# vlaxose/jstsp19

Measured on AMD Instinct MI355X. Metric: channel-estimates/sec (batched MC) at Nt=Nr=64,K=64; NMSE vs ref, higher is better.
Workload: dtype c32 (storage and results fp32 complex; big contractions as split-f16 MFMA with fp32 accumulation, fp32-equivalent); 1 GPU; proposed_algorithm approximate Imax=100, Nt=Nr=64 Nrf=8 K=64 L=8 (N=64 M=4096 Gr=64 G2=512); Imax=100, outputs=S,Y,convergence_error, pilots=per-trial (B per trial), parallelism=trials sharded, dp1

## Files before the change

jstsp19_amd/csrc/admm.hip:

```cpp
#include "common.h"
#include <algorithm>

namespace jstsp {

struct c2 { float2 a, b; };

__device__ __forceinline__ c2 ld2(const float2 *p, long long i)
{
    const float4 v = *reinterpret_cast<const float4 *>(p + i);
    c2 r; r.a = make_float2(v.x, v.y); r.b = make_float2(v.z, v.w); return r;
}
__device__ __forceinline__ void st2(float2 *p, long long i, const c2 &v)
{
    *reinterpret_cast<float4 *>(p + i) = make_float4(v.a.x, v.a.y, v.b.x, v.b.y);
}

__device__ __forceinline__ double wave_sum(double v)
{
    for (int o = 32; o > 0; o >>= 1) v += __shfl_xor(v, o);
    return v;
}

__device__ __forceinline__ double block_sum(double v, double *sh)
{
    v = wave_sum(v);
    __syncthreads();
    if ((threadIdx.x & 63) == 0) sh[threadIdx.x >> 6] = v;
    __syncthreads();
    return sh[0] + sh[1] + sh[2] + sh[3];
}

__global__ __launch_bounds__(256) void form_z_kernel(long long nm, const float2 *X, const float2 *V1,
                                                     const TrialParams *prm, float2 *Z)
{
    const int t = blockIdx.y;
    const TrialParams p = prm[t];
    const long long base = (long long)t * nm;
    const long long stride = (long long)gridDim.x * 256 * 2;
    const bool vec = (nm & 1) == 0;
    for (long long i = ((long long)blockIdx.x * 256 + threadIdx.x) * 2; i < nm; i += stride) {
        if (vec && i + 1 < nm) {
            const c2 x = ld2(X, base + i), v = ld2(V1, base + i);
            c2 z;
            z.a = make_float2(admm_z(p, x.a.x, v.a.x), admm_z(p, x.a.y, v.a.y));
            z.b = make_float2(admm_z(p, x.b.x, v.b.x), admm_z(p, x.b.y, v.b.y));
            st2(Z, base + i, z);
        } else {
            for (long long j = i; j < nm && j < i + 2; ++j) {
                const float2 x = X[base + j], v = V1[base + j];
                Z[base + j] = make_float2(admm_z(p, x.x, v.x), admm_z(p, x.y, v.y));
            }
        }
    }
}

__device__ __forceinline__ void upd_x_one(float2 &x, float2 &v1, const float2 v2, const float2 c,
                                          const float2 xs, const float2 y, const float2 sy,
                                          const float id, const TrialParams &p, float2 &k)
{
    const float tx = (y.x + c.x) + xs.x, ty = (y.y + c.y) + xs.y;
    const float bx = (v1.x + sy.x) + v2.x + mul2(p.rho, p.rho_lo, tx);
    const float by = (v1.y + sy.y) + v2.y + mul2(p.rho, p.rho_lo, ty);
    x = make_float2(bx * id, by * id);
    k = make_float2((fmaf(-p.irho, v2.x, x.x) - p.irho_lo * v2.x) - c.x, (fmaf(-p.irho, v2.y, x.y) - p.irho_lo * v2.y) - c.y);
    v1 = make_float2(admm_v1(p, v1.x, y.x, x.x), admm_v1(p, v1.y, y.y, x.y));
}

__global__ __launch_bounds__(256) void update_x_kernel(long long nm, float2 *X, float2 *V1,
                                                       const float2 *V2, const float2 *C,
                                                       const float2 *Xs, const float2 *Y,
                                                       const float2 *subY, const float *invD,
                                                       const TrialParams *prm, float2 *K)
{
    const int t = blockIdx.y;
    const TrialParams p = prm[t];
    const long long base = (long long)t * nm;
    const long long stride = (long long)gridDim.x * 256 * 2;
    const bool vec = (nm & 1) == 0;
    for (long long i = ((long long)blockIdx.x * 256 + threadIdx.x) * 2; i < nm; i += stride) {
        if (vec && i + 1 < nm) {
            c2 x, k, v1 = ld2(V1, base + i);
            const c2 v2 = ld2(V2, base + i), c = ld2(C, base + i), xs = ld2(Xs, base + i),
                     y = ld2(Y, base + i), sy = ld2(subY, base + i);
            const float2 id = *reinterpret_cast<const float2 *>(invD + base + i);
            upd_x_one(x.a, v1.a, v2.a, c.a, xs.a, y.a, sy.a, id.x, p, k.a);
            upd_x_one(x.b, v1.b, v2.b, c.b, xs.b, y.b, sy.b, id.y, p, k.b);
            st2(X, base + i, x); st2(V1, base + i, v1); st2(K, base + i, k);
        } else {
            for (long long j = i; j < nm && j < i + 2; ++j) {
                float2 x, k, v1 = V1[base + j];
                upd_x_one(x, v1, V2[base + j], C[base + j], Xs[base + j], Y[base + j], subY[base + j],
                          invD[base + j], p, k);
                X[base + j] = x; V1[base + j] = v1; K[base + j] = k;
            }
        }
    }
}

__device__ __forceinline__ void upd_c_one(const float2 x, const float2 xs, float2 &v2, float2 &c, const TrialParams &p)
{
    const float dx = x.x - xs.x, dy = x.y - xs.y;
    const float tx = fmaf(-p.irho, v2.x, dx) - p.irho_lo * v2.x, ty = fmaf(-p.irho, v2.y, dy) - p.irho_lo * v2.y;
    c = make_float2(mul2(p.c_coef, p.c_lo, tx), mul2(p.c_coef, p.c_lo, ty));
    const float ux = c.x - dx, uy = c.y - dy;
    v2 = make_float2(fmaf(p.rho, ux, v2.x) + p.rho_lo * ux, fmaf(p.rho, uy, v2.y) + p.rho_lo * uy);
}

__global__ __launch_bounds__(256) void update_c_kernel(long long nm, const float2 *X, const float2 *Xs,
                                                       float2 *V2, float2 *C, const TrialParams *prm)
{
    const int t = blockIdx.y;
    const TrialParams p = prm[t];
    const long long base = (long long)t * nm;
    const long long stride = (long long)gridDim.x * 256 * 2;
    const bool vec = (nm & 1) == 0;
    for (long long i = ((long long)blockIdx.x * 256 + threadIdx.x) * 2; i < nm; i += stride) {
        if (vec && i + 1 < nm) {
            const c2 x = ld2(X, base + i), xs = ld2(Xs, base + i);
            c2 v2 = ld2(V2, base + i), c;
            upd_c_one(x.a, xs.a, v2.a, c.a, p);
            upd_c_one(x.b, xs.b, v2.b, c.b, p);
            st2(C, base + i, c); st2(V2, base + i, v2);
        } else {
            for (long long j = i; j < nm && j < i + 2; ++j) {
                float2 v2 = V2[base + j], c;
                upd_c_one(X[base + j], Xs[base + j], v2, c, p);
                C[base + j] = c; V2[base + j] = v2;
            }
        }
    }
}

__global__ __launch_bounds__(256) void inv_d_kernel(long long nm, const float *Omega, float scale,
                                                    const TrialParams *prm, float *invD)
{
    const int t = blockIdx.y;
    const double add = (double)scale * ((double)prm[t].rho + (double)prm[t].rho_lo);
    const long long base = (long long)t * nm;
    const long long stride = (long long)gridDim.x * 256;
    for (long long i = (long long)blockIdx.x * 256 + threadIdx.x; i < nm; i += stride)
        invD[base + i] = (float)(1.0 / ((double)Omega[base + i] + add));
}

__device__ __forceinline__ float soft1(float v, float t)
{
    const float m = fmaxf(fabsf(v) - t, 0.f);
    return (v > 0.f) ? m : ((v < 0.f) ? -m : 0.f);
}

template <int NT>
__device__ __forceinline__ double block_sum_nt(double v, double *sh)
{
    v = wave_sum(v);
    __syncthreads();
    if ((threadIdx.x & 63) == 0) sh[threadIdx.x >> 6] = v;
    __syncthreads();
    double s = 0;
#pragma unroll
    for (int w = 0; w < NT / 64; ++w) s += sh[w];
    return s;
}
template <int NT>
__global__ __launch_bounds__(NT) void step_v_kernel(int g, const float2 *Res, const float2 *RRes,
                                                    float2 *V, float2 *S, const int32_t *rank,
                                                    int cnt, const TrialParams *prm, double *ce3,
                                                    int Imax, int it, float2 *RV, uint32_t *zero8)
{
    __shared__ double sh[NT / 64];
    const int t = blockIdx.x;
    const long long base = (long long)t * g;
    double num = 0, den_re = 0, den_im = 0, vprev = 0;
    constexpr int UN = 8;
    for (int i0 = threadIdx.x; i0 < g; i0 += NT * UN) {
        float2 r[UN], rr[UN], v[UN];
#pragma unroll
        for (int u = 0; u < UN; ++u) {
            const int i = min(i0 + u * NT, g - 1);
            r[u] = Res[base + i]; rr[u] = RRes[base + i]; v[u] = V[base + i];
        }
#pragma unroll
        for (int u = 0; u < UN; ++u)
            if (i0 + u * NT < g) {
                num += (double)r[u].x * r[u].x + (double)r[u].y * r[u].y;
                den_re += (double)r[u].x * rr[u].x + (double)r[u].y * rr[u].y;
                den_im += (double)r[u].x * rr[u].y - (double)r[u].y * rr[u].x;
                vprev += (double)v[u].x * v[u].x + (double)v[u].y * v[u].y;
            }
    }
    num = block_sum_nt<NT>(num, sh);
    den_re = block_sum_nt<NT>(den_re, sh);
    den_im = block_sum_nt<NT>(den_im, sh);
    vprev = block_sum_nt<NT>(vprev, sh);
    const double dd = den_re * den_re + den_im * den_im;
    const float ax = (float)(num * den_re / dd);
    const float ay = (float)(-num * den_im / dd);
    const float thr = prm[t].tauS_rho;
    for (int i0 = threadIdx.x; i0 < g; i0 += NT * UN) {
        float2 r[UN], v[UN], rr[UN], rv[UN];
        int rk[UN];
#pragma unroll
        for (int u = 0; u < UN; ++u) {
            const int i = min(i0 + u * NT, g - 1);
            r[u] = Res[base + i]; v[u] = V[base + i];
            if (RV) { rr[u] = RRes[base + i]; rv[u] = RV[base + i]; }
            rk[u] = rank ? rank[base + i] : 0;
        }
#pragma unroll
        for (int u = 0; u < UN; ++u) {
            const int i = i0 + u * NT;
            if (i >= g) break;
            float2 vn = v[u];
            vn.x += ax * r[u].x - ay * r[u].y;
            vn.y += ax * r[u].y + ay * r[u].x;
            V[base + i] = vn;
            if (RV) {
                float2 rn = rv[u];
                rn.x += ax * rr[u].x - ay * rr[u].y;
                rn.y += ax * rr[u].y + ay * rr[u].x;
                RV[base + i] = rn;
            }
            float2 sv = make_float2(soft1(vn.x, thr), soft1(vn.y, thr));
            if (rank && rk[u] >= cnt) sv = make_float2(0.f, 0.f);
            S[base + i] = sv;
        }
    }
    if (zero8 && threadIdx.x < 8) zero8[(size_t)threadIdx.x * gridDim.x + t] = 0u;
    if (ce3 && threadIdx.x == 0) {
        const double a2 = (double)ax * ax + (double)ay * ay;
        ce3[(long long)t * 3 * Imax + 2 * Imax + it] = a2 * num / vprev;
    }
}

__global__ __launch_bounds__(256) void soft_kernel(int g, const float2 *V, float2 *S,
                                                   const int32_t *rank, int cnt, const TrialParams *prm)
{
    const int t = blockIdx.y;
    const long long base = (long long)t * g;
    const float thr = prm[t].tauS_rho;
    for (int i = blockIdx.x * 256 + threadIdx.x; i < g; i += gridDim.x * 256) {
        const float2 v = V[base + i];
        float2 s = make_float2(soft1(v.x, thr), soft1(v.y, thr));
        if (rank && rank[base + i] >= cnt) s = make_float2(0.f, 0.f);
        S[base + i] = s;
    }
}

__global__ void rank_init_kernel(long long n, int32_t *rank)
{
    const long long i = (long long)blockIdx.x * 256 + threadIdx.x;
    if (i < n) rank[i] = 0x7fffffff;
}
__global__ void rank_scatter_kernel(int g, const int32_t *indx, int32_t *rank)
{
    const int t = blockIdx.y;
    const int p = blockIdx.x * 256 + threadIdx.x;
    if (p < g) {
        const int pos = indx[(long long)t * g + p] - 1;
        if (pos >= 0 && pos < g) atomicMin(&rank[(long long)t * g + pos], p);
    }
}

__global__ void ce_ratio_kernel(int batch, const float *lamV1, const float *lamV2, const float *lamX,
                                double *ce, int Imax, int it)
{
    const int t = blockIdx.x * 256 + threadIdx.x;
    if (t < batch) {
        ce[(long long)t * 3 * Imax + it] = (double)lamV1[t] / (double)lamX[t];
        ce[(long long)t * 3 * Imax + Imax + it] = (double)lamV2[t] / (double)lamX[t];
    }
}

static inline dim3 ew_grid(long long nm, int batch)
{
    long long blocks = (nm / 2 + 255) / 256;
    if (blocks < 1) blocks = 1;
    const long long cap = (2048 + batch - 1) / batch;
    if (blocks > cap) blocks = cap < 1 ? 1 : cap;
    return dim3((unsigned)blocks, (unsigned)batch);
}

int launch_form_z(jstsp_ctx *ctx, long long nm, int batch, const float2 *X, const float2 *V1,
                  const TrialParams *prm, float2 *Z)
{
    hipLaunchKernelGGL(form_z_kernel, ew_grid(nm, batch), dim3(256), 0, ctx->stream, nm, X, V1, prm, Z);
    JSTSP_HIP(hipGetLastError());
    return 0;
}
int launch_update_x(jstsp_ctx *ctx, long long nm, int batch, float2 *X, float2 *V1, const float2 *V2,
                    const float2 *C, const float2 *Xs, const float2 *Y, const float2 *subY,
                    const float *invD, const TrialParams *prm, float2 *K)
{
    hipLaunchKernelGGL(update_x_kernel, ew_grid(nm, batch), dim3(256), 0, ctx->stream, nm, X, V1, V2, C,
                       Xs, Y, subY, invD, prm, K);
    JSTSP_HIP(hipGetLastError());
    return 0;
}
int launch_update_c(jstsp_ctx *ctx, long long nm, int batch, const float2 *X, const float2 *Xs,
                    float2 *V2, float2 *C, const TrialParams *prm)
{
    hipLaunchKernelGGL(update_c_kernel, ew_grid(nm, batch), dim3(256), 0, ctx->stream, nm, X, Xs, V2, C,
                       prm);
    JSTSP_HIP(hipGetLastError());
    return 0;
}
int launch_step_v(jstsp_ctx *ctx, int g, int batch, const float2 *Res, const float2 *RRes, float2 *V,
                  float2 *S, const int32_t *rank, int cnt, const TrialParams *prm, double *ce3,
                  int Imax, int it, float2 *RV, int waves8, uint32_t *zero8)
{
    if (g >= 8192 && waves8)
        hipLaunchKernelGGL(step_v_kernel<512>, dim3(batch), dim3(512), 0, ctx->stream, g, Res, RRes, V, S, rank,
                           cnt, prm, ce3, Imax, it, RV, zero8);
    else if (g >= 8192)
        hipLaunchKernelGGL(step_v_kernel<1024>, dim3(batch), dim3(1024), 0, ctx->stream, g, Res, RRes, V, S, rank,
                           cnt, prm, ce3, Imax, it, RV, zero8);
    else
        hipLaunchKernelGGL(step_v_kernel<256>, dim3(batch), dim3(256), 0, ctx->stream, g, Res, RRes, V, S, rank,
                           cnt, prm, ce3, Imax, it, RV, zero8);
    JSTSP_HIP(hipGetLastError());
    return 0;
}
int launch_soft(jstsp_ctx *ctx, int g, int batch, const float2 *V, float2 *S, const int32_t *rank,
                int cnt, const TrialParams *prm)
{
    hipLaunchKernelGGL(soft_kernel, dim3((g + 255) / 256, batch), dim3(256), 0, ctx->stream, g, V, S,
                       rank, cnt, prm);
    JSTSP_HIP(hipGetLastError());
    return 0;
}
int launch_inv_d(jstsp_ctx *ctx, long long nm, int batch, const float *Omega, float scale,
                 const TrialParams *prm, float *invD)
{
    hipLaunchKernelGGL(inv_d_kernel, ew_grid(nm * 2, batch), dim3(256), 0, ctx->stream, nm, Omega, scale,
                       prm, invD);
    JSTSP_HIP(hipGetLastError());
    return 0;
}
int launch_rank_from_index(jstsp_ctx *ctx, int g, int batch, const int32_t *indx, int32_t *rank)
{
    const long long n = (long long)g * batch;
    hipLaunchKernelGGL(rank_init_kernel, dim3((unsigned)((n + 255) / 256)), dim3(256), 0, ctx->stream, n,
                       rank);
    hipLaunchKernelGGL(rank_scatter_kernel, dim3((g + 255) / 256, batch), dim3(256), 0, ctx->stream, g,
                       indx, rank);
    JSTSP_HIP(hipGetLastError());
    return 0;
}
__global__ __launch_bounds__(256) void eye_minus_kernel(int n, long long total, const float2 *Q, float2 *P)
{
    for (long long e = (long long)blockIdx.x * 256 + threadIdx.x; e < total; e += (long long)gridDim.x * 256) {
        const int r = (int)(e % ((long long)n * n));
        const float2 q = Q[e];
        P[e] = make_float2(((r % n) == (r / n) ? 1.f : 0.f) - q.x, -q.y);
    }
}
int launch_eye_minus(jstsp_ctx *ctx, int n, int count, const float2 *Q, float2 *P)
{
    const long long total = (long long)count * n * n;
    hipLaunchKernelGGL(eye_minus_kernel, dim3((unsigned)std::min<long long>((total + 255) / 256, 2048)), dim3(256), 0,
                       ctx->stream, n, total, Q, P);
    JSTSP_HIP(hipGetLastError());
    return 0;
}

int launch_ce_ratio(jstsp_ctx *ctx, int batch, const float *lamV1, const float *lamV2, const float *lamX,
                    double *ce, int Imax, int it)
{
    hipLaunchKernelGGL(ce_ratio_kernel, dim3((batch + 255) / 256), dim3(256), 0, ctx->stream, batch,
                       lamV1, lamV2, lamX, ce, Imax, it);
    JSTSP_HIP(hipGetLastError());
    return 0;
}

}
```

jstsp19_amd/csrc/common.h:

```cpp
#pragma once
#include <hip/hip_runtime.h>
#include <cstdint>
#include <cstdio>
#include <cstdarg>
#include <string>
#include <vector>
#include <map>
#include "../../include/jstsp.h"

namespace jstsp {

void set_error(const char *fmt, ...);

#define JSTSP_HIP(call)                                                                  \
    do {                                                                                 \
        hipError_t e_ = (call);                                                          \
        if (e_ != hipSuccess) {                                                          \
            jstsp::set_error("%s failed: %s (%s:%d)", #call, hipGetErrorString(e_),      \
                             __FILE__, __LINE__);                                        \
            return (int)e_;                                                              \
        }                                                                                \
    } while (0)

#define JSTSP_TRY(expr)                                                                  \
// ... 95 lines not shown
    const float ys = y + xs;
    const float s = (v1 + sy) + mul2(p.rho, p.rho_lo, ys) + mul2(p.omr, p.omr_lo, v2);
    return fmaf(s, rh, s * rl);
}
__device__ __forceinline__ void admm_invd(const TrialParams &p, float om, float &rh, float &rl)
{
    const float a = 2.f * p.rho, al = 2.f * p.rho_lo;
    const float dh = om + a;
    const float bb = dh - om;
    const float dl = ((om - (dh - bb)) + (a - bb)) + al;
    rh = __builtin_amdgcn_rcpf(dh);
    rl = rh * (fmaf(-dh, rh, 1.f) - dl * rh);
}
__device__ __forceinline__ float admm_k(const TrialParams &p, float x, float v2) { return fmaf(p.omir, v2, x) + p.omir_lo * v2; }
__device__ __forceinline__ float admm_v1(const TrialParams &p, float v1, float y, float x)
{
    const float d = y - x;
    return fmaf(p.rho, d, v1) + p.rho_lo * d;
}
__device__ __forceinline__ float admm_z(const TrialParams &p, float x, float v1) { return fmaf(-p.irho, v1, x) - p.irho_lo * v1; }
#endif
#endif

struct Arena {
    char *base = nullptr;
    size_t cap = 0, off = 0;
    int reserve(size_t bytes);
    void reset() { off = 0; }
    template <class T> T *get(size_t n) {
        size_t bytes = (n * sizeof(T) + 255) & ~size_t(255);
        if (off + bytes > cap) return nullptr;
        T *p = reinterpret_cast<T *>(base + off);
        off += bytes;
        return p;
    }
    void release();
};

struct ProfileSlot {
    int launches = 0;
    std::vector<std::pair<hipEvent_t, hipEvent_t>> pending;
    double total_ms = 0;
};

}

struct jstsp_ctx {
    int device = 0;
    hipStream_t stream = nullptr;
    bool own_stream = false;
    jstsp::Arena arena;
    bool profiling = false;
    std::map<std::string, jstsp::ProfileSlot> prof;
    std::vector<hipEvent_t> event_pool;
    int num_cus = 256;
    void *pinned = nullptr;
    size_t pinned_cap = 0, pinned_off = 0;
    hipEvent_t pinned_done = nullptr;
    bool pinned_pending = false;
    uint32_t *diag = nullptr;
    unsigned *lz_mismatch = nullptr;
    void *hpin = nullptr;
    size_t hpin_cap = 0;
    hipEvent_t hpin_done = nullptr;
    bool hpin_pending = false;
    int dict_block_hint = 0;
    int last_dict_block = 0;
    int fused_fallbacks = 0;
    float2 *unit = nullptr;
    double2 *unit64 = nullptr;
    jstsp_ctx *helper = nullptr;
    hipStream_t side[2] = {nullptr, nullptr};
    hipStream_t cu_stream[4] = {nullptr, nullptr, nullptr, nullptr};
    int cu_state = 0;
    hipStream_t bj_stream[3] = {nullptr, nullptr, nullptr};
    hipEvent_t bj_ev[6] = {nullptr, nullptr, nullptr, nullptr, nullptr, nullptr};
    hipEvent_t ev[10] = {nullptr, nullptr, nullptr, nullptr, nullptr, nullptr, nullptr, nullptr, nullptr, nullptr};
};

namespace jstsp {

struct GemmDesc {
    const float2 *A; long long sAt, sAi, sAk; int conjA;
    const float2 *B; long long sBt, sBk, sBj; int conjB;
    const float2 *B2;
    float2 *C; long long sCt; int ldc;
    const float2 *D; long long sDt; int ldd;
    float alpha, beta;
    int m, n, k, batch;
    int splitk; long long sCsplit;
    int epi;
    const TrialParams *prm;
    float2 *e_rw0, *e_w1, *e_w2, *e_w3;
    const float2 *e_r0, *e_r1, *e_r2, *e_r3;
    const float *e_f0;
    int epi_store_c;
    uint32_t *amax_x, *amax_v1, *amax_z;
    uint32_t *amax_out;
    int force_m64;
    float2 *C_lo;
    int herm_upper;
    int sa_mode;
    const float *sa_lr, *sa_lt;
    float sa_rho, sa_thr;
};
__device__ __forceinline__ float sadmm_den(float lr, float lt, float rho) { return fmaf(lr, lt, -rho); }
__device__ __forceinline__ float sadmm_dual1(float z, float r, float s, float rho) { return fmaf(rho, r - s, z); }
__device__ __forceinline__ float sadmm_soft1(float r, float z, float ir, float thr)
{
    const float v = fmaf(ir, z, r);
    const float m = fmaxf(fabsf(v) - thr, 0.f);
    return (v > 0.f) ? m : ((v < 0.f) ? -m : 0.f);
}
__device__ __forceinline__ float sadmm_rhs1(float z, float s, float a, float rho) { return fmaf(-rho, s, z) + a; }
enum { EPI_NONE = 0, EPI_UPDATE_C = 1, EPI_UPDATE_X = 2, EPI_SADMM = 3 };
enum { GEMM_MISC = 0, GEMM_CORRELATE = 1, GEMM_SYNTH = 2, GEMM_GRAM = 3 };
int launch_cgemm(jstsp_ctx *ctx, const GemmDesc &d, int tag = GEMM_MISC);

struct HPack {
    uint4 *data = nullptr;
    uint32_t *bmax = nullptr;
    int KS = 0, JT = 0, count = 0;
    long long st = 0;
};
struct HGemmDesc {
    const float2 *A; long long sAt, sAk;
    const uint32_t *amax;
    const uint4 *Bp; long long sPt;
    const uint32_t *bmax; int sbmax;
    int KS, JT;
    float2 *C; long long sCt; int ldc;
    int m, n, k, batch;
    int epi;
    const TrialParams *prm;
    const float2 *e_r0;
    float2 *e_rw0;
    uint32_t *amax_v2;
    const uint4 *Ap; long long sApt; int aKS;
    int herm_upper;
    int map_tb, map_tt;
};
int hermitian_fill_lower(jstsp_ctx *ctx, float2 *G, long long sGt, int n, int count);
int launch_hgram(jstsp_ctx *ctx, const float2 *Z, long long sZt, int rows, int cols, int count, int nsplit,
                 const uint32_t *amax, float2 *Gpart, const float2 *Z2 = nullptr,
                 const TrialParams *zprm = nullptr,
                 bool norm_only = false);
int launch_hgram3(jstsp_ctx *ctx, const float2 *X, const float2 *V1, long long sZt, int rows, int cols, int count, int nsplit,
                  const uint32_t *xmax, const uint32_t *vmax, const uint32_t *zmax, const TrialParams *prm, float2 *Gz,
                  float2 *Gx, float2 *Gv);
size_t hgemm_pack_bytes(int Kd, int J, int count);
bool hgemm_pair_shape(int m, int n, int batch);
int hgemm_absmax(jstsp_ctx *ctx, const float2 *X, long long n, long long sXt, int count, uint32_t *amax);
int hgemm_pack(jstsp_ctx *ctx, HPack &p, Arena &ar, const float2 *B, long long sBt, long long sBk, long long sBj,
               int conj, int Kd, int J, int count, long long n_contig, const uint32_t *bmax_known = nullptr);
int hgemm_repack(jstsp_ctx *ctx, const HPack &p, const float2 *B, long long sBt, long long sBk, long long sBj, int conj,
                 int Kd, int J, const uint32_t *bmax);
int launch_hgemm(jstsp_ctx *ctx, const HGemmDesc &d, const char *prof_name = nullptr);
bool use_hgemm(long long m, long long n, long long k);

enum { EIG_SVT_Q = 0, EIG_LMAX = 1, EIG_VECS = 2 };
int launch_eig(jstsp_ctx *ctx, int mode, int n, int batch, const float2 *Gpart, long long sGt,
               int nsplit, long long sGs, const TrialParams *prm, const float *tau,
               float2 *Q, float *lam_out, float2 *Vg);
bool eig_needs_global_v(int n);
int launch_eig_large(jstsp_ctx *ctx, int mode, int n, int batch, const float2 *Gpart, long long sGt, int nsplit,
                     long long sGs, const TrialParams *prm, const float *tau, float2 *Q, float *lam_out);
int launch_eig_fast(jstsp_ctx *ctx, int mode, int n, int batch, const float2 *Gpart, long long sGt, int nsplit,
                    long long sGs, const TrialParams *prm, const float *tau, float2 *Q, float *lam_out,
                    float2 *Uwarm, int warm);
int launch_eig128(jstsp_ctx *ctx, int n, int batch, const float2 *Gpart, long long sGt, int nsplit, long long sGs,
                  const TrialParams *prm, const float *tau, float2 *Q, float2 *Uwarm = nullptr, int warm = 0,
                  int max_sweeps = 16, float stop_level = 0.f);
int eig_fast_ne(int n);
struct LanczosWarm {
    float2 *x = nullptr;
    int *state = nullptr;
    unsigned *mismatch = nullptr;
    int ne = 0;
    int call = 0;
};
int lanczos_ne(int n);
int launch_lmax(jstsp_ctx *ctx, int n, int batch, const float2 *Gpart, long long sGt, int nsplit, long long sGs,
                float *lam_out, bool lanczos = false, const LanczosWarm *lw = nullptr, int first = 0);

int launch_form_z(jstsp_ctx *ctx, long long nm, int batch, const float2 *X, const float2 *V1,
                  const TrialParams *prm, float2 *Z);
int launch_update_x(jstsp_ctx *ctx, long long nm, int batch, float2 *X, float2 *V1,
                    const float2 *V2, const float2 *C, const float2 *Xs, const float2 *Y,
                    const float2 *subY, const float *invD, const TrialParams *prm, float2 *K);
int launch_update_c(jstsp_ctx *ctx, long long nm, int batch, const float2 *X, const float2 *Xs,
                    float2 *V2, float2 *C, const TrialParams *prm);
int launch_step_v(jstsp_ctx *ctx, int g, int batch, const float2 *Res, const float2 *RRes,
                  float2 *V, float2 *S, const int32_t *rank, int cnt, const TrialParams *prm,
                  double *ce3, int Imax, int it, float2 *RV = nullptr, int waves8 = 0,
                  uint32_t *zero8 = nullptr);
int launch_soft(jstsp_ctx *ctx, int g, int batch, const float2 *V, float2 *S, const int32_t *rank,
                int cnt, const TrialParams *prm);
int launch_inv_d(jstsp_ctx *ctx, long long nm, int batch, const float *Omega, float scale2rho,
                 const TrialParams *prm, float *invD);
int launch_rank_from_index(jstsp_ctx *ctx, int g, int batch, const int32_t *indx, int32_t *rank);
int launch_eye_minus(jstsp_ctx *ctx, int n, int count, const float2 *Q, float2 *P);
int launch_ce_ratio(jstsp_ctx *ctx, int batch, const float *lamV1, const float *lamV2,
                    const float *lamX, double *ce, int Imax, int it);

void prof_begin(jstsp_ctx *ctx, const char *name);
void prof_end(jstsp_ctx *ctx, const char *name);

}
```

jstsp19_amd/csrc/fused.hip:

```cpp
#include "solver_common.h"
#include <algorithm>
#include <cstdlib>
#include <cstdio>

namespace jstsp {
namespace {

typedef _Float16 half8 __attribute__((ext_vector_type(8)));
typedef _Float16 half4 __attribute__((ext_vector_type(4)));
typedef float f32x4 __attribute__((ext_vector_type(4)));

constexpr int FPAD = 128;

__device__ __host__ inline int fscale_exp(uint32_t amax_bits)
{
    const int be = (int)((amax_bits >> 23) & 0xff);
    if (be == 0 || be == 255) return 0;
    return 13 - (be - 127);
}
__device__ __forceinline__ void fsplit(float x, _Float16 &h, _Float16 &l)
{
    h = (_Float16)x;
    l = (_Float16)(x - (float)h);
}
typedef unsigned int u32x4 __attribute__((ext_vector_type(4)));
typedef unsigned int u32x2 __attribute__((ext_vector_type(2)));
__device__ __forceinline__ u32x4 negu(u32x4 u) { return u ^ 0x80008000u; }
template <class T> __device__ __forceinline__ T ldg(const void *base, uint32_t boff)
{
    return *reinterpret_cast<const T *>(reinterpret_cast<const char *>(base) + boff);
}
template <class T> __device__ __forceinline__ T ldg_nt(const void *base, uint32_t boff)
{
    return __builtin_nontemporal_load(reinterpret_cast<const T *>(reinterpret_cast<const char *>(base) + boff));
}
typedef float f32x2 __attribute__((ext_vector_type(2)));
__device__ __forceinline__ float2 ldg_nt2(const void *base, uint32_t boff)
{
    const f32x2 v = ldg_nt<f32x2>(base, boff);
    return make_float2(v.x, v.y);
}
__device__ __forceinline__ void stg_nt2(void *base, uint32_t boff, float2 v)
{
    __builtin_nontemporal_store(f32x2{v.x, v.y}, reinterpret_cast<f32x2 *>(reinterpret_cast<char *>(base) + boff));
}
template <class T> __device__ __forceinline__ void stg(void *base, uint32_t boff, T v)
{
    *reinterpret_cast<T *>(reinterpret_cast<char *>(base) + boff) = v;
}
__device__ __forceinline__ f32x4 mma(u32x4 a, u32x4 b, f32x4 c)
{
    return __builtin_amdgcn_mfma_f32_16x16x32_f16(__builtin_bit_cast(half8, a), __builtin_bit_cast(half8, b), c, 0, 0, 0);
}

__global__ __launch_bounds__(256) void pack_bf_kernel(const float2 *B, long long sBt, int G2, int M, const uint32_t *bmax,
                                                      int sbmax, uint4 *out, long long sOut)
{
    const int t = blockIdx.y;
    const int G8 = G2 >> 3;
    const long long per_tile = 32ll * G8;
    const long long idx = (long long)blockIdx.x * 256 + threadIdx.x;
    if (idx >= (long long)(M / 32) * per_tile) return;
    const int tile = (int)(idx / per_tile);
    int rem = (int)(idx % per_tile);
    const int g8 = rem % G8; rem /= G8;
    const int r = rem & 3, mq = rem >> 2;
    const int m = tile * 32 + 4 * mq + r;
    const float s = ldexpf(1.f, fscale_exp(bmax[(long long)t * sbmax]));
    half8 pl[4];
#pragma unroll
    for (int c = 0; c < 8; ++c) {
        const float2 x = B[(long long)t * sBt + (8 * g8 + c) + (long long)G2 * m];
        _Float16 h, l;
        fsplit(x.x * s, h, l); pl[0][c] = h; pl[1][c] = l;
        fsplit(x.y * s, h, l); pl[2][c] = h; pl[3][c] = l;
    }
    uint4 *o = out + (long long)t * sOut + (long long)tile * (16ll * G2);
    const int blk = g8 >> 1, g8i = g8 & 1;
#pragma unroll
    for (int p = 0; p < 4; ++p) o[(((long long)(blk * 4 + p) * 8 + mq) * 2 + g8i) * 4 + r] = *reinterpret_cast<uint4 *>(&pl[p]);
}

__global__ __launch_bounds__(256) void toeplitz_probe_kernel(const float2 *B, long long sBt, int G2, int M, uint32_t cand, uint32_t *mism)
{
    const uint32_t idx = blockIdx.x * 256u + threadIdx.x;
    uint32_t bad = 0;
    if (idx < (uint32_t)G2 * (uint32_t)M) {
        const int m = (int)(idx / (uint32_t)G2), g = (int)(idx - (uint32_t)m * (uint32_t)G2);
        const uint2 *b = reinterpret_cast<const uint2 *>(B) + (long long)blockIdx.y * sBt;
        const uint2 x = b[idx];
#pragma unroll
        for (int c = 0; c < 5; ++c) {
            const int gt = 16 << c, ld = g >> (4 + c);
            if (!((cand >> c) & 1u) || ld == 0 || m < ld) continue;
            const uint2 y = b[idx - (uint32_t)gt - (uint32_t)G2];
            if (x.x != y.x || x.y != y.y) bad |= 1u << c;
        }
    }
#pragma unroll
    for (int o = 32; o > 0; o >>= 1) bad |= __shfl_xor(bad, o);
    if ((threadIdx.x & 63) == 0 && (bad & ~__atomic_load_n(mism, __ATOMIC_RELAXED))) atomicOr(mism, bad);
}

__global__ __launch_bounds__(256) void toeplitz_verify_kernel(const float2 *B, long long sBt, int G2, int M, int c, uint32_t *mism)
{
    const uint32_t q = blockIdx.x * 256u + threadIdx.x;
    const uint32_t qpc = (uint32_t)G2 >> 2;
    uint32_t bad = 0;
    if (q < qpc * (uint32_t)M) {
        const int m = (int)(q / qpc), g = 4 * (int)(q - (uint32_t)m * qpc);
        const int gt = 16 << c, ld = g >> (4 + c);
        if (ld >= 1 && m >= ld) {
            const uint4 *b = reinterpret_cast<const uint4 *>(reinterpret_cast<const uint2 *>(B) + (long long)blockIdx.y * sBt);
            const uint32_t e = (uint32_t)g + (uint32_t)G2 * (uint32_t)m;
            const uint4 x0 = b[e >> 1], x1 = b[(e >> 1) + 1];
            const uint32_t f = e - (uint32_t)gt - (uint32_t)G2;
            const uint4 y0 = b[f >> 1], y1 = b[(f >> 1) + 1];
            if (x0.x != y0.x || x0.y != y0.y || x0.z != y0.z || x0.w != y0.w || x1.x != y1.x || x1.y != y1.y || x1.z != y1.z ||
                x1.w != y1.w)
                bad = 1u << c;
        }
    }
#pragma unroll
    for (int o = 32; o > 0; o >>= 1) bad |= __shfl_xor(bad, o);
    if ((threadIdx.x & 63) == 0 && (bad & ~__atomic_load_n(mism, __ATOMIC_RELAXED))) atomicOr(mism, bad);
}

__global__ __launch_bounds__(256) void pack_e_kernel(const float2 *B, long long sBt, int G2, int M, int gt, int ecols, int ehalo,
                                                     const uint32_t *bmax, int sbmax, uint4 *out, long long sOut)
{
    const int t = blockIdx.y;
    const int G8t = gt >> 3, L = G2 / gt;
    const long long idx = (long long)blockIdx.x * 256 + threadIdx.x;
    if (idx >= (long long)G8t * ecols) return;
    const int g8 = (int)(idx % G8t), j = (int)(idx / G8t);
    int row0 = 8 * g8, m = j - ehalo;
    bool live = true;
    if (m < 0) {
        const int jh = -m;
        int ld = 1;
        while (ld * (ld + 1) / 2 < jh) ++ld;
        live = ld < L;
        const int c = -(jh - ld * (ld - 1) / 2);
        m = c + ld; row0 += ld * gt;
    }
    const float s = ldexpf(1.f, fscale_exp(bmax[(long long)t * sbmax]));
    half8 pl[4];
#pragma unroll
    for (int c = 0; c < 8; ++c) {
        const float2 x = live ? B[(long long)t * sBt + (row0 + c) + (long long)G2 * m] : make_float2(0.f, 0.f);
        _Float16 h, l;
        fsplit(x.x * s, h, l); pl[0][c] = h; pl[1][c] = l;
        fsplit(x.y * s, h, l); pl[2][c] = h; pl[3][c] = l;
    }
    uint4 *o = out + (long long)t * sOut;
#pragma unroll
    for (int p = 0; p < 4; ++p) o[(long long)(p * G8t + g8) * ecols + j] = *reinterpret_cast<uint4 *>(&pl[p]);
}

__host__ __device__ inline int eswz(int x) { return (((x >> 1) & 3) << 1) | ((x >> 3) & 1); }

__global__ __launch_bounds__(256) void pack_e2_kernel(const float2 *B, long long sBt, int G2, int M, const uint32_t *bmax, int sbmax,
                                                      uint4 *out, long long sOut, float2 *Bdl)
{
    const int t = blockIdx.y;
    const int idx = blockIdx.x * 256 + threadIdx.x;
    if (idx < G2 * 8)
        Bdl[(long long)t * G2 * 8 + idx] = B[(long long)t * sBt + (idx >> 3) + (long long)G2 * (idx & 7)];
    if (idx >= (M + 8) * 8) return;
    const int o = idx & 7, cc = idx >> 3, m = cc - 7;
    const bool live = m >= 0 && m < M;
    const float s = ldexpf(1.f, fscale_exp(bmax[(long long)t * sbmax]));
    half8 pl[4];
#pragma unroll
    for (int c = 0; c < 8; ++c) {
        const float2 x = live ? B[(long long)t * sBt + (8 * o + c) + (long long)G2 * m] : make_float2(0.f, 0.f);
        _Float16 h, l;
        fsplit(x.x * s, h, l); pl[0][c] = h; pl[1][c] = l;
        fsplit(x.y * s, h, l); pl[2][c] = h; pl[3][c] = l;
    }
    uint4 *dst = out + (long long)t * sOut;
#pragma unroll
    for (int p = 0; p < 4; ++p) dst[((long long)p * (M + 8) + cc) * 8 + (o ^ eswz(cc))] = *reinterpret_cast<uint4 *>(&pl[p]);
}

__device__ __forceinline__ void xs_delta(const float2 *W, const float2 *Bdl, int G2, int m, int r, float2 *out)
{
    __shared__ float2 part[4][64];
    const int lane = threadIdx.x & 63, wv = threadIdx.x >> 6;
    const int g0 = 64 * (m + 1), cnt = G2 - g0;
    float2 a = make_float2(0.f, 0.f), a2 = a;
    const int per = (cnt + 15) / 16, lo = min(g0 + (4 * r + wv) * per, G2), hi = min(lo + per, G2);
    int g = lo;
    for (; g + 8 <= hi; g += 8) {
        float2 w[8], b[8];
#pragma unroll
        for (int u = 0; u < 8; ++u) { w[u] = W[lane + 64ll * (g + u)]; b[u] = Bdl[(g + u) * 8 + m]; }
#pragma unroll
        for (int u = 0; u < 8; u += 2) {
            a.x = fmaf(w[u].x, b[u].x, fmaf(-w[u].y, b[u].y, a.x)); a.y = fmaf(w[u].x, b[u].y, fmaf(w[u].y, b[u].x, a.y));
            a2.x = fmaf(w[u + 1].x, b[u + 1].x, fmaf(-w[u + 1].y, b[u + 1].y, a2.x));
            a2.y = fmaf(w[u + 1].x, b[u + 1].y, fmaf(w[u + 1].y, b[u + 1].x, a2.y));
        }
    }
    for (; g < hi; ++g) {
        const float2 w0 = W[lane + 64ll * g], b0 = Bdl[g * 8 + m];
        a.x = fmaf(w0.x, b0.x, fmaf(-w0.y, b0.y, a.x)); a.y = fmaf(w0.x, b0.y, fmaf(w0.y, b0.x, a.y));
    }
    part[wv][lane] = make_float2(a.x + a2.x, a.y + a2.y);
    __syncthreads();
    if (wv == 0) {
        const float2 p0 = part[0][lane], p1 = part[1][lane], p2 = part[2][lane], p3 = part[3][lane];
        out[lane + 64 * m] = make_float2((p0.x + p1.x) + (p2.x + p3.x), (p0.y + p1.y) + (p2.y + p3.y));
    }
}

__global__ __launch_bounds__(256) void pack_as_kernel(const float2 *W, long long sWt, int G2, const uint32_t *wmax, uint4 *out,
                                                      long long sOut, const float2 *Bd, long long sBd, float2 *XsD)
{
    const int t = blockIdx.y;
    if ((int)blockIdx.x >= G2 / 32) {
        const int e = (int)blockIdx.x - G2 / 32;
        xs_delta(W + (long long)t * sWt, Bd + (long long)t * sBd, G2, e >> 2, e & 3, XsD + (long long)t * 2048 + (e & 3) * 512);
        return;
    }
    const int idx = blockIdx.x * 256 + threadIdx.x;
    if (idx >= (G2 / 32) * 256) return;
    const int lane = idx & 63, nb = (idx >> 6) & 3, ks = idx >> 8;
    const int n = 16 * nb + (lane & 15), g0 = 32 * ks + 8 * (lane >> 4);
    const float s = ldexpf(1.f, fscale_exp(wmax[t]));
    half8 pl[4];
#pragma unroll
    for (int v = 0; v < 8; ++v) {
        const float2 x = W[(long long)t * sWt + n + 64ll * (g0 + v)];
        _Float16 h, l;
        fsplit(x.x * s, h, l); pl[0][v] = h; pl[1][v] = l;
        fsplit(x.y * s, h, l); pl[2][v] = h; pl[3][v] = l;
    }
    uint4 *o = out + (long long)t * sOut + (long long)((ks * 4 + nb) * 4) * 64 + lane;
#pragma unroll
    for (int p = 0; p < 4; ++p) o[p * 64] = *reinterpret_cast<uint4 *>(&pl[p]);
}

__global__ __launch_bounds__(256) void pack_wq_kernel(const float2 *Q, uint4 *out)
{
    const int t = blockIdx.x;
    const float2 *q = Q + (long long)t * 4096;
    for (int idx = threadIdx.x; idx < 512; idx += 256) {
        const int lane = idx & 63, nb = (idx >> 6) & 3, ks = idx >> 8;
        const int n = 16 * nb + (lane & 15), c0 = 32 * ks + 8 * (lane >> 4);
        half8 pl[4];
#pragma unroll
        for (int v = 0; v < 8; ++v) {
            const float2 x = q[n + 64 * (c0 + v)];
            _Float16 h, l;
            fsplit(((n == c0 + v) ? 1.f : 0.f) * 8192.f - x.x * 8192.f, h, l); pl[0][v] = h; pl[1][v] = l;
            fsplit(-x.y * 8192.f, h, l); pl[2][v] = h; pl[3][v] = l;
        }
        uint4 *o = out + (long long)t * 2048 + (long long)((ks * 4 + nb) * 4) * 64 + lane;
#pragma unroll
        for (int p = 0; p < 4; ++p) o[p * 64] = *reinterpret_cast<uint4 *>(&pl[p]);
    }
}

__global__ __launch_bounds__(256) void reduce_parts_kernel(const float4 *P, int parts, long long n4, float4 *out)
{
    const int t = blockIdx.y;
    const long long i = (long long)blockIdx.x * 256 + threadIdx.x;
    if (i >= n4) return;
    const float4 *p = P + (long long)t * parts * n4 + i;
    const float4 a0 = p[0];
    double ax = a0.x, ay = a0.y, az = a0.z, aw = a0.w;
    for (int s = 1; s < parts; ++s) {
        const float4 b = p[(long long)s * n4];
        ax += b.x; ay += b.y; az += b.z; aw += b.w;
    }
    out[(long long)t * n4 + i] = make_float4((float)ax, (float)ay, (float)az, (float)aw);
}
// ... 536 lines not shown
            ev2[s] = *reinterpret_cast<const float2 *>(sp_ + 2 * SFLD);  esy[s] = *reinterpret_cast<const float2 *>(sp_ + 3 * SFLD);
            eid[s] = *reinterpret_cast<const float *>(stag + SINV + (4 * q + s) * ICOL + c16 * 4);
        }
        __syncthreads();
        f32x4 xr = kh ? ar[1] : ar[0], xi = kh ? ai[1] : ai[0];
        {
            const f32x4 *x4 = reinterpret_cast<const f32x4 *>(pex);
            const f32x4 orr = x4[(w * 2 + 0) * 64 + l], oi = x4[(w * 2 + 1) * 64 + l];
            xr += orr; xi += oi;
        }
        half4 kf[4];
#pragma unroll
        for (int s = 0; s < 4; ++s) {
            const uint32_t ix = ebase + 512u * (uint32_t)(m0 + s);
            float2 xs = make_float2(xr[s] * sxs, xi[s] * sxs);
            const bool lead = m0 == 0 && kh == 0 && 4 * q + s < 2 * GB - 1;
            if (lead) {
                const float2 d0 = ldg<float2>(XsDt, ix), d1 = ldg<float2>(XsDt, ix + 4096), d2 = ldg<float2>(XsDt, ix + 8192),
                             d3 = ldg<float2>(XsDt, ix + 12288);
                xs.x += (d0.x + d1.x) + (d2.x + d3.x); xs.y += (d0.y + d1.y) + (d2.y + d3.y);
            }
            const float2 v2 = make_float2(admm_v2(prm, ev2[s].x, ex[s].x, xs.x), admm_v2(prm, ev2[s].y, ex[s].y, xs.y));
            float rh = eid[s], rl = 0.f;
            if (d.inv_is_omega) admm_invd(prm, eid[s], rh, rl);
            const float2 x = make_float2(admm_x2(prm, ev1[s].x, ey[s].x, esy[s].x, v2.x, xs.x, rh, rl),
                                         admm_x2(prm, ev1[s].y, ey[s].y, esy[s].y, v2.y, xs.y, rh, rl));
            const float2 kk = make_float2(admm_k(prm, x.x, v2.x), admm_k(prm, x.y, v2.y));
            const float2 v1 = make_float2(admm_v1(prm, ev1[s].x, ey[s].x, x.x), admm_v1(prm, ev1[s].y, ey[s].y, x.y));
            stg_nt2(V2t, ix, v2); stg_nt2(Xt, ix, x); stg_nt2(V1t, ix, v1);
            const float2 zn = make_float2(admm_z(prm, x.x, v1.x), admm_z(prm, x.y, v1.y));
            if (Zot) stg_nt2(Zot, ix, zn);
            if (Yot) stg(Yot, ix, ey[s]);
            if (lead) stg(Kft, ix, kk);
            v2mx = fmaxf(v2mx, fmaxf(fabsf(v2.x), fabsf(v2.y)));
            xmx = fmaxf(xmx, fmaxf(fabsf(x.x), fabsf(x.y)));
            v1mx = fmaxf(v1mx, fmaxf(fabsf(v1.x), fabsf(v1.y)));
            zmx = fmaxf(zmx, fmaxf(fabsf(zn.x), fabsf(zn.y)));
            kmx = fmaxf(kmx, fmaxf(fabsf(kk.x), fabsf(kk.y)));
            _Float16 h, lo;
            fsplit(kk.x * sk, h, lo); kf[0][s] = h; kf[1][s] = lo;
            fsplit(kk.y * sk, h, lo); kf[2][s] = h; kf[3][s] = lo;
        }
#pragma unroll
        for (int p = 0; p < 4; ++p)
            *reinterpret_cast<half4 *>(xch + ((nb * 6 + p) * 64 + l) * 16 + kh * 8) = kf[p];
        *reinterpret_cast<half4 *>(xch + ((nb * 6 + 4) * 64 + l) * 16 + kh * 8) = -kf[0];
        *reinterpret_cast<half4 *>(xch + ((nb * 6 + 5) * 64 + l) * 16 + kh * 8) = -kf[1];
        __syncthreads();
        const int tn = tile0 + min(i + 1, tpw - 1);
        typedef short s16x4 __attribute__((ext_vector_type(4)));
        typedef __attribute__((address_space(3))) s16x4 lds_s16x4;
        auto *lbase = (__attribute__((address_space(3))) unsigned char *)lds;
#pragma unroll
        for (int gb = 0; gb < GB; ++gb) {
            const int blk = GB * ws + gb, ld = blk >> 2, jp = 2 * (blk & 3);
            int cB = cB0 - ld;
            asm volatile("" : "+v"(cB));
            const uint32_t tr0 = (uint32_t)((i & 1) * EBUF) + cB * 128 + 16 * ((jp + ((c16 >> 1) & 1)) ^ eswz(cB)) + (c16 & 1) * 8;
            u32x4 bf[4];
#pragma unroll
            for (int p = 0; p < 4; ++p) {
                const uint32_t o_ = tr0 + p * EPL;
                const u32x2 lo_ = __builtin_bit_cast(u32x2, __builtin_amdgcn_ds_read_tr16_b64_v4i16((lds_s16x4 *)(lbase + o_)));
                const u32x2 hi_ = __builtin_bit_cast(u32x2, __builtin_amdgcn_ds_read_tr16_b64_v4i16((lds_s16x4 *)(lbase + o_ + 2048)));
                bf[p] = u32x4{lo_.x, lo_.y, hi_.x, hi_.y};
            }
#pragma unroll
            for (int n2 = 0; n2 < 4; ++n2) {
                const unsigned char *kp = xch + (n2 * 6 * 64 + l) * 16;
                u32x4 k0 = *reinterpret_cast<const u32x4 *>(kp), k1 = *reinterpret_cast<const u32x4 *>(kp + 1024);
                const u32x4 k2 = *reinterpret_cast<const u32x4 *>(kp + 2048), k3 = *reinterpret_cast<const u32x4 *>(kp + 3072);
                f32x4 tr = mma(bf[0], k0, f32x4{0.f, 0.f, 0.f, 0.f}), ti = mma(bf[0], k2, f32x4{0.f, 0.f, 0.f, 0.f});
                tr = mma(bf[0], k1, tr); ti = mma(bf[0], k3, ti);
                tr = mma(bf[1], k0, tr); ti = mma(bf[1], k2, ti);
                k0 = *reinterpret_cast<const u32x4 *>(kp + 4096); k1 = *reinterpret_cast<const u32x4 *>(kp + 5120);
                tr = mma(bf[2], k2, tr); ti = mma(bf[2], k0, ti);
                tr = mma(bf[2], k3, tr); ti = mma(bf[2], k1, ti);
                tr = mma(bf[3], k2, tr); ti = mma(bf[3], k0, ti);
                {
                    const int grp = 4 * gb + n2;
                    if (grp >= 6 && grp - 6 < 12) F64_STORE(grp - 6, (i + 1) & 1, rf[((grp - 6) >> 2) & 1][(grp - 6) & 3])
                    if (grp < 12) F64_LOAD(grp, tn, rf[(grp >> 2) & 1][grp & 3])
                }
                pr[gb][n2] += tr; pi[gb][n2] += ti;
                __builtin_amdgcn_sched_barrier(0);
            }
        }
        {
            constexpr int NG = 4 * GB;
#pragma unroll
            for (int pc = (NG > 6 ? NG - 6 : 0); pc < 12; ++pc) {
                if (pc >= NG) F64_LOAD(pc, tn, rf[(pc >> 2) & 1][pc & 3])
                F64_STORE(pc, (i + 1) & 1, rf[(pc >> 2) & 1][pc & 3])
            }
        }
        __builtin_amdgcn_sched_barrier(0);
        F64_WQLOAD()
        __syncthreads();
    }
#undef F64_LOAD
#undef F64_STORE
#undef F64_FLD
#undef F64_J
#undef F64_WQLOAD
    float2 *po = d.Ppart + ((long long)t * d.parts + part) * (64ll * G2);
#pragma unroll
    for (int gb = 0; gb < GB; ++gb)
#pragma unroll
        for (int n2 = 0; n2 < 4; ++n2)
#pragma unroll
            for (int s = 0; s < 4; ++s) {
                const int g = 16 * GB * w + 16 * gb + 4 * q + s;
                po[64ll * g + 16 * n2 + c16] = make_float2(pr[gb][n2][s] * sp, pi[gb][n2][s] * sp);
            }
#pragma unroll
    for (int o = 32; o > 0; o >>= 1) {
        kmx = fmaxf(kmx, __shfl_xor(kmx, o)); xmx = fmaxf(xmx, __shfl_xor(xmx, o)); v1mx = fmaxf(v1mx, __shfl_xor(v1mx, o));
        zmx = fmaxf(zmx, __shfl_xor(zmx, o)); v2mx = fmaxf(v2mx, __shfl_xor(v2mx, o));
    }
    if (l == 0) {
        if (d.kmax_out) atomicMax(&d.kmax_out[t], __float_as_uint(kmx));
        if (d.xmax) atomicMax(&d.xmax[t], __float_as_uint(xmx));
        if (d.v1max) atomicMax(&d.v1max[t], __float_as_uint(v1mx));
        if (d.zmax) atomicMax(&d.zmax[t], __float_as_uint(zmx));
        if (d.v2max) atomicMax(&d.v2max[t], __float_as_uint(v2mx));
        if (d.ovf && !(kmx * sk < 60000.f)) atomicOr(&d.ovf[t], 1u);
    }
}

}

bool fused_shape_ok(int N, int M, int G2, int parts)
{
    return N == 64 && G2 >= 128 && G2 <= 512 && G2 % 128 == 0 && parts > 0 && M % (32 * parts) == 0;
}

static void compact_dims(int M, int G2, int gt, int *ecols, int *ehalo)
{
    const int L = G2 / gt;
    *ehalo = ((L * (L - 1) / 2 + 3) / 4) * 4;
    *ecols = *ehalo + M;
}

size_t fused_bytes(int M, int G2, int nB, int batch, int parts)
{
    int ec, eh;
    compact_dims(M, G2, 16, &ec, &eh);
    return rnd256((size_t)nB * (M / 32) * 16 * G2 * sizeof(uint4)) + rnd256((size_t)batch * (G2 / 32) * 1024 * sizeof(uint4)) +
           rnd256((size_t)batch * parts * 64 * G2 * sizeof(float2)) + rnd256((size_t)batch * sizeof(uint32_t)) + rnd256((size_t)batch * 2048 * sizeof(uint4)) +
           rnd256((size_t)nB * 4 * (G2 / 16) * ec * sizeof(uint4)) + 5 * rnd256((size_t)batch * 512 * sizeof(float2)) +
           rnd256((size_t)nB * G2 * 8 * sizeof(float2)) + 512;
}

int fused_probe_toeplitz(jstsp_ctx *ctx, Arena &ar, const float2 *B, long long sBt, int G2, int M, int nB, int *gt)
{
    *gt = 0;
    uint32_t *flag = ar.get<uint32_t>(1);
    JSTSP_REQUIRE(flag, JSTSP_E_NOMEM, "fused pass: workspace exhausted");
    JSTSP_REQUIRE((long long)G2 * M < (1ll << 31), JSTSP_E_UNSUPPORTED, "fused pass: dictionary too large");
    uint32_t cand = 0;
    for (int c = 0; c < 5; ++c)
        if (G2 % (16 << c) == 0 && 2 * (16 << c) <= G2) cand |= 1u << c;
    const unsigned nblk = (unsigned)(((long long)G2 * M + 255) / 256);
    for (int step = 0; step < (nB > 1 ? 2 : 1) && cand; ++step) {
        JSTSP_HIP(hipMemsetAsync(flag, 0, sizeof(uint32_t), ctx->stream));
        if (step && sBt % 2 == 0)
            hipLaunchKernelGGL(toeplitz_verify_kernel, dim3((nblk + 3) / 4, nB), dim3(256), 0, ctx->stream, B, sBt, G2, M,
                               31 - __builtin_clz(cand), flag);
        else
            hipLaunchKernelGGL(toeplitz_probe_kernel, dim3(nblk, step ? nB : 1), dim3(256), 0, ctx->stream, B, sBt, G2, M, cand, flag);
        JSTSP_HIP(hipGetLastError());
        uint32_t bad = ~0u;
        JSTSP_HIP(hipMemcpyAsync(&bad, flag, sizeof(uint32_t), hipMemcpyDeviceToHost, ctx->stream));
        JSTSP_HIP(hipStreamSynchronize(ctx->stream));
        cand &= ~bad;
        cand &= cand ? (~cand + 1u) : 0u;
    }
    if (cand) *gt = 16 << (31 - __builtin_clz(cand));
    return 0;
}

__global__ __launch_bounds__(256) void toeplitz_gram_kernel(const float2 *B, long long sBt, int G2, int M, int gt, const float2 *G0,
                                                            const float2 *G0lo, float2 *G, float2 *Glo)
{
    const int t = blockIdx.y;
    const int idx = blockIdx.x * 256 + threadIdx.x;
    if (idx >= G2 * G2) return;
    const int r = idx % G2, c = idx / G2;
    const int ld = r / gt, g = r - ld * gt, l2 = c / gt, g2 = c - l2 * gt;
    if (ld > l2) return;
    const int d = l2 - ld;
    const float2 *b = B + (long long)t * sBt;
    const long long i0 = (long long)t * gt * G2 + g + (long long)gt * (d * gt + g2);
    double vr = (double)G0[i0].x + (G0lo ? (double)G0lo[i0].x : 0.0), vi = (double)G0[i0].y + (G0lo ? (double)G0lo[i0].y : 0.0);
    auto mac = [&](float2 x, float2 y, double sgn) {
        vr += sgn * ((double)x.x * y.x + (double)x.y * y.y);
        vi += sgn * ((double)x.y * y.x - (double)x.x * y.y);
    };
    for (int m = 0; m < d; ++m) mac(b[g + (long long)G2 * m], b[d * gt + g2 + (long long)G2 * m], -1.0);
    for (int u = M - ld; u < M; ++u) mac(b[g + (long long)G2 * u], b[g2 + (long long)G2 * (u - d)], -1.0);
    for (int m = 0; m < l2; ++m) mac(b[r + (long long)G2 * m], b[c + (long long)G2 * m], 1.0);
    if (r == c) vi = 0.0;
    const float hr = (float)vr, hi = (float)vi;
    float2 *o = G + (long long)t * G2 * G2;
    o[r + (long long)G2 * c] = make_float2(hr, hi);
    if (ld < l2) o[c + (long long)G2 * r] = make_float2(hr, -hi);
    if (Glo) {
        float2 *ol = Glo + (long long)t * G2 * G2;
        const float lr = (float)(vr - (double)hr), li = (float)(vi - (double)hi);
        ol[r + (long long)G2 * c] = make_float2(lr, li);
        if (ld < l2) ol[c + (long long)G2 * r] = make_float2(lr, -li);
    }
}

int toeplitz_gram_assemble(jstsp_ctx *ctx, const float2 *B, long long sBt, int G2, int M, int gt, int nB, const float2 *G0,
                           const float2 *G0lo, float2 *G, float2 *Glo)
{
    hipLaunchKernelGGL(toeplitz_gram_kernel, dim3((unsigned)((G2 * G2 + 255) / 256), nB), dim3(256), 0, ctx->stream, B, sBt, G2, M, gt,
                       G0, G0lo, G, Glo);
    JSTSP_HIP(hipGetLastError());
    return 0;
}

int fused_alloc(Arena &ar, FusedWS &f, int M, int G2, int nB, int batch, int parts, int gt, int v2)
{
    f.parts = parts;
    f.sBf = (long long)(M / 32) * 16 * G2;
    f.sAS = (long long)(G2 / 32) * 1024;
    f.gt = gt;
    f.v2 = (gt == 64 && v2) ? 1 : 0;
    if (f.v2) {
        f.ecols = M + 8; f.ehalo = 7;
        f.sEc = 4ll * f.ecols * 8;
        f.Ec = ar.get<uint4>((size_t)nB * f.sEc);
        f.XsD = ar.get<float2>((size_t)batch * 2048);
        f.Kf = ar.get<float2>((size_t)batch * 512);
        f.Bdl = ar.get<float2>((size_t)nB * G2 * 8);
        JSTSP_REQUIRE(f.XsD && f.Kf && f.Bdl, JSTSP_E_NOMEM, "fused pass: workspace exhausted");
    } else if (gt) {
        compact_dims(M, G2, gt, &f.ecols, &f.ehalo);
        f.sEc = 4ll * (gt / 8) * f.ecols;
        f.Ec = ar.get<uint4>((size_t)nB * f.sEc);
    } else
        f.Bf = ar.get<uint4>((size_t)nB * f.sBf);
    f.ASp = ar.get<uint4>((size_t)batch * f.sAS);
    f.Ppart = ar.get<float2>((size_t)batch * parts * 64 * G2);
    f.ovf = ar.get<uint32_t>(batch);
    f.Wqp = ar.get<uint4>((size_t)batch * 2048);
    JSTSP_REQUIRE((f.Bf || f.Ec) && f.ASp && f.Ppart && f.ovf && f.Wqp, JSTSP_E_NOMEM, "fused pass: workspace exhausted");
    return 0;
}

int fused_pack_b(jstsp_ctx *ctx, FusedWS &f, const float2 *B, long long sBt, int G2, int M, int nB, const uint32_t *bmax)
{
    f.Bsrc = B; f.sBsrc = sBt;
    if (f.v2) {
        hipLaunchKernelGGL(pack_e2_kernel, dim3((unsigned)((std::max(M + 8, G2) * 8 + 255) / 256), nB), dim3(256), 0, ctx->stream, B, sBt, G2, M,
                           bmax, 1, f.Ec, f.sEc, f.Bdl);
        JSTSP_HIP(hipGetLastError());
        f.sBdl = sBt ? (long long)G2 * 8 : 0;
        return 0;
    }
    if (f.gt) {
        const long long n = (long long)(f.gt / 8) * f.ecols;
        hipLaunchKernelGGL(pack_e_kernel, dim3((unsigned)((n + 255) / 256), nB), dim3(256), 0, ctx->stream, B, sBt, G2, M, f.gt,
                           f.ecols, f.ehalo, bmax, 1, f.Ec, f.sEc);
        JSTSP_HIP(hipGetLastError());
        return 0;
    }
    const long long n = (long long)(M / 32) * 16 * (G2 / 4);
    hipLaunchKernelGGL(pack_bf_kernel, dim3((unsigned)((n + 255) / 256), nB), dim3(256), 0, ctx->stream, B, sBt, G2, M, bmax, 1,
                       f.Bf, f.sBf);
    JSTSP_HIP(hipGetLastError());
    return 0;
}

int fused_pack_as(jstsp_ctx *ctx, const FusedWS &f, const float2 *W, long long sWt, int G2, int M, int batch, const uint32_t *wmax)
{
    hipLaunchKernelGGL(pack_as_kernel, dim3((G2 / 32) + (f.v2 ? 4 * (G2 / 64 - 1) : 0), batch), dim3(256), 0, ctx->stream, W, sWt, G2, wmax,
                       f.ASp, f.sAS, f.Bdl, f.sBdl, f.XsD);
    JSTSP_HIP(hipGetLastError());
    return 0;
}

template <int GB> static int launch_fused64(jstsp_ctx *ctx, const FusedDesc &d)
{
    const size_t sh = 2 * 20480 + 24576 + 8 * (4 * 16 * 128 + 16 * 80) + 16384;
    const int grid = ((d.batch + 7) / 8) * 8 * d.parts;
    JSTSP_HIP(hipFuncSetAttribute((const void *)fused_pass64_kernel<GB>, hipFuncAttributeMaxDynamicSharedMemorySize, (int)sh));
    hipLaunchKernelGGL((fused_pass64_kernel<GB>), dim3(grid), dim3(512), sh, ctx->stream, d);
    return 0;
}

template <int GB, bool YIN, bool TOEP> static int launch_fused_gb(jstsp_ctx *ctx, const FusedDesc &d)
{
    const size_t sh = (size_t)32 * (128 * GB * 8 + FPAD) + 24576;
    const int grid = ((d.batch + 7) / 8) * 8 * d.parts;
    JSTSP_HIP(hipFuncSetAttribute((const void *)fused_pass_kernel<GB, YIN, TOEP>, hipFuncAttributeMaxDynamicSharedMemorySize, (int)sh));
    hipLaunchKernelGGL((fused_pass_kernel<GB, YIN, TOEP>), dim3(grid), dim3(512), sh, ctx->stream, d);
    return 0;
}

template <bool YIN, bool TOEP> static int launch_fused_y(jstsp_ctx *ctx, const FusedDesc &d)
{
    switch (d.G2 / 128) {
    case 1: return launch_fused_gb<1, YIN, TOEP>(ctx, d);
    case 2: return launch_fused_gb<2, YIN, TOEP>(ctx, d);
    case 3: return launch_fused_gb<3, YIN, TOEP>(ctx, d);
    default: return launch_fused_gb<4, YIN, TOEP>(ctx, d);
    }
}

int launch_fused_pass(jstsp_ctx *ctx, const FusedDesc &d)
{
    JSTSP_REQUIRE(fused_shape_ok(64, d.M, d.G2, d.parts), JSTSP_E_UNSUPPORTED, "fused pass: shape");
    JSTSP_REQUIRE(d.Ec ? (d.gsh >= 4 && d.gsh <= 8) : d.Bf != nullptr, JSTSP_E_UNSUPPORTED, "fused pass: dictionary image");
    prof_begin(ctx, "fused_pass");
    int rc = 0;
    if (d.v2) {
// ... 39 lines not shown
```

jstsp19_amd/csrc/hgemm.hip:

```cpp
#include "solver_common.h"
#include <type_traits>

namespace jstsp {

typedef _Float16 half8 __attribute__((ext_vector_type(8)));
typedef float f32x16 __attribute__((ext_vector_type(16)));
typedef unsigned int u32x4 __attribute__((ext_vector_type(4)));

namespace {

constexpr int HBK = 32;
constexpr int FLUSH = 8;
constexpr float LO_SCALE = 1.f, LO_INV = 1.f;

__device__ __host__ inline int scale_exp(uint32_t amax_bits)
{
    const int be = (int)((amax_bits >> 23) & 0xff);
    if (be == 0 || be == 255) return 0;
    return 13 - (be - 127);
}

__device__ __forceinline__ void split2(float x, _Float16 &h, _Float16 &l)
{
    h = (_Float16)x;
    l = (_Float16)((x - (float)h) * LO_SCALE);
}

__global__ __launch_bounds__(256) void absmax_kernel(long long n2, const float *X, long long sXt, uint32_t *amax)
{
    const int t = blockIdx.y;
    const float *p = X + (long long)t * sXt;
    float m = 0.f;
    const bool vec = ((sXt & 3) == 0) && ((n2 & 3) == 0) && (((uintptr_t)X & 15) == 0);
    if (vec) {
        const float4 *p4 = reinterpret_cast<const float4 *>(p);
        for (long long i = (long long)blockIdx.x * 256 + threadIdx.x; i < n2 / 4; i += (long long)gridDim.x * 256) {
            const float4 v = p4[i];
            m = fmaxf(fmaxf(m, fmaxf(fabsf(v.x), fabsf(v.y))), fmaxf(fabsf(v.z), fabsf(v.w)));
        }
    } else {
        for (long long i = (long long)blockIdx.x * 256 + threadIdx.x; i < n2; i += (long long)gridDim.x * 256)
            m = fmaxf(m, fabsf(p[i]));
    }
    for (int o = 32; o > 0; o >>= 1) m = fmaxf(m, __shfl_xor(m, o));
    __shared__ float sm[4];
    if ((threadIdx.x & 63) == 0) sm[threadIdx.x >> 6] = m;
    __syncthreads();
    if (threadIdx.x == 0)
        atomicMax(&amax[t], __float_as_uint(fmaxf(fmaxf(sm[0], sm[1]), fmaxf(sm[2], sm[3]))));
}

__global__ __launch_bounds__(256) void pack_b_kernel(const float2 *B, long long sBt, long long sBk, long long sBj,
                                                     int conj, int Kd, int J, int KS, int JT, const uint32_t *bmax,
                                                     uint4 *out)
{
    const int t = blockIdx.y;
    const long long idx = (long long)blockIdx.x * 256 + threadIdx.x;
    if (idx >= (long long)JT * KS * 64) return;
    const int lane = (int)(idx & 63);
    const long long blk = idx >> 6;
    const int ks = (int)(blk % KS), jt = (int)(blk / KS);
    const int j = jt * 32 + (lane & 31), k0 = ks * 16 + 8 * (lane >> 5);
    const float s = ldexpf(1.f, scale_exp(bmax[t]));
    const float sg = conj ? -s : s;
    half8 rh, rl, ih, il;
#pragma unroll
    for (int v = 0; v < 8; ++v) {
        float2 x = make_float2(0.f, 0.f);
        if (j < J && k0 + v < Kd) x = B[(long long)t * sBt + (long long)(k0 + v) * sBk + (long long)j * sBj];
        _Float16 h, l;
        split2(x.x * s, h, l); rh[v] = h; rl[v] = l;
        split2(x.y * sg, h, l); ih[v] = h; il[v] = l;
    }
    uint4 *o = out + (((long long)t * JT + jt) * KS + ks) * 256 + lane;
    o[0] = *reinterpret_cast<uint4 *>(&rh);
    o[64] = *reinterpret_cast<uint4 *>(&rl);
    o[128] = *reinterpret_cast<uint4 *>(&ih);
    o[192] = *reinterpret_cast<uint4 *>(&il);
}

__device__ __forceinline__ half8 as_half8(uint4 u) { return *reinterpret_cast<half8 *>(&u); }
__device__ __forceinline__ half8 neg_half8(uint4 u)
{
    u.x ^= 0x80008000u; u.y ^= 0x80008000u; u.z ^= 0x80008000u; u.w ^= 0x80008000u;
    return *reinterpret_cast<half8 *>(&u);
}

__device__ __forceinline__ bool block_to_trial_tile(const HGemmDesc &d, int tiles, int &t, int &tile)
{
    const int bid = blockIdx.x;
    const int xcd = bid & 7, slot = bid >> 3;
    if (d.map_tb == 0) {
        t = (slot / tiles) * 8 + xcd;
        tile = slot % tiles;
        return t < d.batch;
    }
    const int per = d.map_tb * d.map_tt;
    const int nbt = (d.batch + d.map_tb - 1) / d.map_tb;
    const int blk = (slot / per) * 8 + xcd, w = slot % per;
    t = (blk % nbt) * d.map_tb + w % d.map_tb;
    tile = (blk / nbt) * d.map_tt + w / d.map_tb;
    return t < d.batch && tile < tiles;
}

template <int EPI, bool APACK, int WJ, bool EVEN = false>
__global__ __launch_bounds__(128 * WJ, WJ == 2 ? 2 : 2) void hgemm_kernel(HGemmDesc d, int tiles_i, int tiles_j)
{
    constexpr int STG = 1024 + 512 * WJ;
    constexpr int NA = (WJ == 2) ? 8 : 4;
    __shared__ uint4 smem[2 * STG];

    const int tiles = tiles_i * tiles_j;
    int t, rem;
    if (!block_to_trial_tile(d, tiles, t, rem)) return;
    const int ti = rem % tiles_i, tj = rem / tiles_i;
    const int i0 = ti * 64, j0 = tj * 32 * WJ;
    if (d.herm_upper && i0 >= j0 + 32 * WJ) return;

    const int tid = threadIdx.x, lane = tid & 63, wave = tid >> 6;
    const int wi = wave & 1, wj = wave >> 1;

    const int ea = scale_exp(d.amax[t]);
    const int eb = scale_exp(d.bmax[(long long)t * d.sbmax]);
    const float sa = ldexpf(1.f, ea);

    const int ai = tid & 63, akg = tid >> 6;
    const bool arow = (i0 + ai) < d.m;
    const float2 *abase = APACK ? nullptr : d.A + (long long)t * d.sAt;
    const float2 *pa = APACK ? nullptr : abase + (arow ? (i0 + ai) : 0) + (long long)(NA * akg) * d.sAk;
    const int a_slot = (WJ == 2) ? ((((ai >> 5) * 2 + (akg >> 1)) * 4) * 64) + (akg & 1) * 32 + (ai & 31)
                                 : ((((ai >> 5) * 2 + (akg >> 2)) * 4) * 64) + ((akg >> 1) & 1) * 32 + (ai & 31);
    const uint4 *pb = d.Bp + (long long)t * d.sPt + ((long long)(tj * WJ) * d.KS) * 256 + lane;
    const int nst = d.KS / 2;
    const int kfull = d.k / HBK;

    struct StgF { float2 a[NA]; uint4 b0, b1, b2, b3; };
    struct StgP { u32x4 a0, a1, a2, a3; uint4 b0, b1, b2, b3; };
    using Stg = typename std::conditional<APACK, StgP, StgF>::type;
    const uint4 *pbw = pb + ((long long)(wave >> 1) * d.KS + (wave & 1)) * 256;
    const uint4 *paw = APACK ? d.Ap + (long long)t * d.sApt + lane +
                                   ((long long)(ti * 2 + (wave >> 1)) * d.KS + (wave & 1)) * 256
                             : nullptr;
    const float sa_m = arow ? sa : 0.f;
    auto load = [&](int s_in, Stg &R) {
        const int s = EVEN ? (s_in < nst ? s_in : 0) : s_in;
        const uint4 *g = pbw + (long long)(2 * s) * 256;
        const u32x4 *gn = reinterpret_cast<const u32x4 *>(g);
        const u32x4 x0 = __builtin_nontemporal_load(gn), x1 = __builtin_nontemporal_load(gn + 64),
                    x2 = __builtin_nontemporal_load(gn + 128), x3 = __builtin_nontemporal_load(gn + 192);
        R.b0 = make_uint4(x0.x, x0.y, x0.z, x0.w); R.b1 = make_uint4(x1.x, x1.y, x1.z, x1.w);
        R.b2 = make_uint4(x2.x, x2.y, x2.z, x2.w); R.b3 = make_uint4(x3.x, x3.y, x3.z, x3.w);
        if constexpr (APACK) {
            const u32x4 *ga = reinterpret_cast<const u32x4 *>(paw + (long long)(2 * s) * 256);
            R.a0 = ga[0]; R.a1 = ga[64]; R.a2 = ga[128]; R.a3 = ga[192];
        } else {
            if (EVEN || s < kfull) {
#pragma unroll
                for (int v = 0; v < NA; ++v) R.a[v] = pa[(long long)(s * HBK + v) * d.sAk];
            } else {
                const int kbase = s * HBK + NA * akg;
#pragma unroll
                for (int v = 0; v < NA; ++v) {
                    const bool ok = kbase + v < d.k;
                    const float2 *p = ok ? pa + (long long)(s * HBK + v) * d.sAk : abase;
                    const float2 x = *p;
                    R.a[v] = ok ? x : make_float2(0.f, 0.f);
                }
            }
        }
    };
    auto store = [&](const Stg &R, uint4 *buf) {
        uint4 *o = buf + 1024 + wave * 256 + lane;
        o[0] = R.b0; o[64] = R.b1; o[128] = R.b2; o[192] = R.b3;
        if constexpr (APACK) {
            u32x4 *q = reinterpret_cast<u32x4 *>(buf + wave * 256 + lane);
            q[0] = R.a0; q[64] = R.a1; q[128] = R.a2; q[192] = R.a3;
        } else {
            half8 rh = {0}, rl = {0}, ih = {0}, il = {0};
#pragma unroll
            for (int v = 0; v < NA; ++v) {
                _Float16 h, l;
                split2(R.a[v].x * sa_m, h, l); rh[v] = h; rl[v] = l;
                split2(R.a[v].y * sa_m, h, l); ih[v] = h; il[v] = l;
            }
            if constexpr (WJ == 2) {
                uint4 *q = buf + a_slot;
                q[0] = *reinterpret_cast<uint4 *>(&rh);
                q[64] = *reinterpret_cast<uint4 *>(&rl);
                q[128] = *reinterpret_cast<uint4 *>(&ih);
                q[192] = *reinterpret_cast<uint4 *>(&il);
            } else {
                uint2 *q = reinterpret_cast<uint2 *>(buf + a_slot) + (akg & 1);
                q[0] = *reinterpret_cast<uint2 *>(&rh);
                q[2 * 64] = *reinterpret_cast<uint2 *>(&rl);
                q[2 * 128] = *reinterpret_cast<uint2 *>(&ih);
                q[2 * 192] = *reinterpret_cast<uint2 *>(&il);
            }
        }
    };

    f32x16 re_h = {0}, re_l = {0}, im_h = {0}, im_l = {0};
    f32x16 Lre = {0}, Lim = {0};
    auto fold = [&]() {
#pragma unroll
        for (int r = 0; r < 16; ++r) {
            Lre[r] += re_h[r] + re_l[r] * LO_INV;
            Lim[r] += im_h[r] + im_l[r] * LO_INV;
            re_h[r] = 0.f; re_l[r] = 0.f; im_h[r] = 0.f; im_l[r] = 0.f;
        }
    };
    auto compute = [&](const uint4 *buf) {
#pragma unroll
        for (int ks = 0; ks < 2; ++ks) {
            const uint4 *fa = buf + ((wi * 2 + ks) * 4) * 64 + lane;
            const uint4 *fb = buf + 1024 + ((wj * 2 + ks) * 4) * 64 + lane;
            const uint4 uar_h = fa[0], uar_l = fa[64], uai_h = fa[128], uai_l = fa[192];
            const half8 br_h = as_half8(fb[0]), br_l = as_half8(fb[64]), bi_h = as_half8(fb[128]), bi_l = as_half8(fb[192]);
            const half8 ar_h = as_half8(uar_h), ar_l = as_half8(uar_l), ai_h = as_half8(uai_h), ai_l = as_half8(uai_l);
            const half8 nai_h = neg_half8(uai_h), nai_l = neg_half8(uai_l);
            re_h = __builtin_amdgcn_mfma_f32_32x32x16_f16(br_h, ar_h, re_h, 0, 0, 0);
            re_l = __builtin_amdgcn_mfma_f32_32x32x16_f16(br_l, ar_h, re_l, 0, 0, 0);
            im_h = __builtin_amdgcn_mfma_f32_32x32x16_f16(bi_h, ar_h, im_h, 0, 0, 0);
            im_l = __builtin_amdgcn_mfma_f32_32x32x16_f16(bi_l, ar_h, im_l, 0, 0, 0);
            re_h = __builtin_amdgcn_mfma_f32_32x32x16_f16(bi_h, nai_h, re_h, 0, 0, 0);
            re_l = __builtin_amdgcn_mfma_f32_32x32x16_f16(br_h, ar_l, re_l, 0, 0, 0);
// ... 690 lines not shown
            const float2 *p = px + (long long)(s * HBK) * rows;
#pragma unroll
            for (int u = 0; u < 8; ++u) { R.x[u] = p[(long long)u * rows]; R.v[u] = p[(long long)u * rows + dv]; }
        } else {
            const int kbase = kbeg + s * HBK + 8 * akg;
#pragma unroll
            for (int u = 0; u < 8; ++u) {
                const int kk = min(kbase + u, cols - 1);
                const long long ix = base + (long long)kk * rows;
                float2 a = X[ix], b = V1[ix];
                if (kbase + u >= kend) { a = make_float2(0.f, 0.f); b = make_float2(0.f, 0.f); }
                R.x[u] = a; R.v[u] = b;
            }
        }
    };
    auto put = [&](uint4 *panel, const float2 *val, float sc) {
        half8 rh, rl, ih, il;
#pragma unroll
        for (int u = 0; u < 8; ++u) {
            _Float16 h, l;
            split2(val[u].x * sc, h, l); rh[u] = h; rl[u] = l + l;
            split2(val[u].y * sc, h, l); ih[u] = h; il[u] = l + l;
        }
        uint4 *q = panel + a_slot;
        q[0] = *reinterpret_cast<uint4 *>(&rh);
        q[64] = *reinterpret_cast<uint4 *>(&rl);
        q[128] = *reinterpret_cast<uint4 *>(&ih);
        q[192] = *reinterpret_cast<uint4 *>(&il);
    };
    auto put_h = [&](uint4 *panel, const float2 *val, float sc) {
        half8 rh, ih;
#pragma unroll
        for (int u = 0; u < 8; ++u) { rh[u] = (_Float16)(val[u].x * sc); ih[u] = (_Float16)(val[u].y * sc); }
        uint4 *q = panel + a_slot;
        q[0] = *reinterpret_cast<uint4 *>(&rh);
        q[128] = *reinterpret_cast<uint4 *>(&ih);
    };
    auto store = [&](const Stg &R) {
        float2 z[8];
#pragma unroll
        for (int u = 0; u < 8; ++u)
            z[u] = make_float2(fmaf(-ir, R.v[u].x, R.x[u].x) - irl * R.v[u].x, fmaf(-ir, R.v[u].y, R.x[u].y) - irl * R.v[u].y);
        if constexpr (NH) { put_h(smem, R.x, sx); put_h(smem + 1024, R.v, sv); }
        else { put(smem, R.x, sx); put(smem + 1024, R.v, sv); }
        put(smem + 2048, z, sz);
    };
    f32x16 re[3], im[3];
#pragma unroll
    for (int g = 0; g < 3; ++g)
#pragma unroll
        for (int r = 0; r < 16; ++r) { re[g][r] = 0.f; im[g][r] = 0.f; }
    auto compute = [&]() {
#pragma unroll
        for (int g = 0; g < 3; ++g) {
            const uint4 *buf = smem + g * 1024;
#pragma unroll
            for (int ks = 0; ks < 2; ++ks) {
                const uint4 *fi = buf + ((wi * 2 + ks) * 4) * 64 + lane;
                const uint4 *fj = buf + ((wj * 2 + ks) * 4) * 64 + lane;
                const half8 ir_h = as_half8(fi[0]), ii_h = as_half8(fi[128]);
                const uint4 ujr_h = fj[0], ujr_l = fj[64], uji_h = fj[128], uji_l = fj[192];
                const half8 jr_h = as_half8(ujr_h), jr_l = as_half8(ujr_l), ji_h = as_half8(uji_h), ji_l = as_half8(uji_l);
                const half8 nji_h = neg_half8(uji_h), nji_l = neg_half8(uji_l);
                re[g] = __builtin_amdgcn_mfma_f32_32x32x16_f16(jr_h, ir_h, re[g], 0, 0, 0);
                im[g] = __builtin_amdgcn_mfma_f32_32x32x16_f16(jr_h, ii_h, im[g], 0, 0, 0);
                re[g] = __builtin_amdgcn_mfma_f32_32x32x16_f16(ji_h, ii_h, re[g], 0, 0, 0);
                im[g] = __builtin_amdgcn_mfma_f32_32x32x16_f16(nji_h, ir_h, im[g], 0, 0, 0);
                if (NH && g < 2) continue;
                re[g] = __builtin_amdgcn_mfma_f32_32x32x16_f16(jr_l, ir_h, re[g], 0, 0, 0);
                im[g] = __builtin_amdgcn_mfma_f32_32x32x16_f16(jr_l, ii_h, im[g], 0, 0, 0);
                re[g] = __builtin_amdgcn_mfma_f32_32x32x16_f16(ji_l, ii_h, re[g], 0, 0, 0);
                im[g] = __builtin_amdgcn_mfma_f32_32x32x16_f16(nji_l, ir_h, im[g], 0, 0, 0);
            }
        }
    };
    if (nst > 0) {
        if constexpr (EVEN) {
            Stg R0, R1;
            load(0, R0);
            load(1, R1);
            store(R0);
            __syncthreads();
            for (int s = 0; s < nst; s += 2) {
                load(s + 2, R0);
                compute();
                __syncthreads();
                store(R1);
                __syncthreads();
                load(s + 3, R1);
                compute();
                __syncthreads();
                store(R0);
                __syncthreads();
            }
        } else {
            Stg R;
            load(0, R);
            store(R);
            __syncthreads();
            for (int s = 0; s < nst; ++s) {
                load(min(s + 1, nst - 1), R);
                compute();
                __syncthreads();
                store(R);
                __syncthreads();
            }
        }
    }
#pragma unroll
    for (int g = 0; g < 3; ++g) herm_symmetrize(re[g], im[g], reinterpret_cast<float2 *>(smem), wi, wj, lane);
    const int gi = wi * 32 + (lane & 31);
    const long long po = ((long long)t * nsplit + split) * rows * rows;
    if (gi < rows) {
        const float ax = ldexpf(1.f, -2 * ex), av = ldexpf(1.f, -2 * ev), az = ldexpf(1.f, -2 * ez);
#pragma unroll
        for (int r = 0; r < 16; ++r) {
            const int gj = wj * 32 + (r & 3) + 8 * (r >> 2) + 4 * (lane >> 5);
            if (gj < rows) {
                const long long o = po + gi + (long long)gj * rows;
                Gx[o] = make_float2(re[0][r] * ax, im[0][r] * ax);
                Gv[o] = make_float2(re[1][r] * av, im[1][r] * av);
                Gz[o] = make_float2(re[2][r] * az, im[2][r] * az);
            }
        }
    }
}

}

bool use_hgemm(long long m, long long n, long long k)
{
    const int mode = tune().h2;
    if (mode == 0) return false;
    if (mode >= 2) return true;
    return m * n * k >= (1ll << 22) && k >= 64 && n >= 64;
}

size_t hgemm_pack_bytes(int Kd, int J, int count)
{
    const size_t KS = 4 * (size_t)((Kd + 63) / 64), JT = 4 * (size_t)((J + 127) / 128);
    return rnd256((size_t)count * JT * KS * 4096) + rnd256((size_t)count * sizeof(uint32_t));
}

int hgemm_absmax(jstsp_ctx *ctx, const float2 *X, long long n, long long sXt, int count, uint32_t *amax)
{
    JSTSP_HIP(hipMemsetAsync(amax, 0, (size_t)count * sizeof(uint32_t), ctx->stream));
    const int gx = (int)std::max<long long>(1, std::min<long long>(2 * n / 4 / 256 / 16, std::max(16, 4096 / std::max(count, 1))));
    absmax_kernel<<<dim3(gx, count), 256, 0, ctx->stream>>>(2 * n, reinterpret_cast<const float *>(X), 2 * sXt, amax);
    JSTSP_HIP(hipGetLastError());
    return 0;
}

int hgemm_pack(jstsp_ctx *ctx, HPack &p, Arena &ar, const float2 *B, long long sBt, long long sBk, long long sBj,
               int conj, int Kd, int J, int count, long long n_contig, const uint32_t *bmax_known)
{
    p.KS = 4 * ((Kd + 63) / 64);
    p.JT = 4 * ((J + 127) / 128);
    p.count = count;
    p.st = (long long)p.JT * p.KS * 256;
    p.data = ar.get<uint4>((size_t)count * p.st);
    p.bmax = ar.get<uint32_t>(count);
    JSTSP_REQUIRE(p.data && p.bmax, JSTSP_E_NOMEM, "workspace exhausted (packed dictionary)");
    if (bmax_known) JSTSP_HIP(hipMemcpyAsync(p.bmax, bmax_known, (size_t)count * sizeof(uint32_t), hipMemcpyDeviceToDevice, ctx->stream));
    else JSTSP_TRY(hgemm_absmax(ctx, B, n_contig, sBt, count, p.bmax));
    const long long slots = (long long)p.JT * p.KS * 64;
    pack_b_kernel<<<dim3((unsigned)((slots + 255) / 256), count), 256, 0, ctx->stream>>>(B, sBt, sBk, sBj, conj, Kd, J,
                                                                                         p.KS, p.JT, p.bmax, p.data);
    JSTSP_HIP(hipGetLastError());
    return 0;
}

int hgemm_repack(jstsp_ctx *ctx, const HPack &p, const float2 *B, long long sBt, long long sBk, long long sBj, int conj,
                 int Kd, int J, const uint32_t *bmax)
{
    const long long slots = (long long)p.JT * p.KS * 64;
    pack_b_kernel<<<dim3((unsigned)((slots + 255) / 256), p.count), 256, 0, ctx->stream>>>(B, sBt, sBk, sBj, conj, Kd, J,
                                                                                           p.KS, p.JT, bmax, p.data);
    JSTSP_HIP(hipGetLastError());
    return 0;
}

int launch_hgram(jstsp_ctx *ctx, const float2 *Z, long long sZt, int rows, int cols, int count, int nsplit,
                 const uint32_t *amax, float2 *Gpart, const float2 *Z2, const TrialParams *zprm, bool norm_only)
{
    JSTSP_REQUIRE(rows > 0 && rows <= 64 && cols > 0 && count > 0 && nsplit > 0, JSTSP_E_SHAPE, "hgram: bad shape");
    const long long grid = (long long)count * nsplit;
    JSTSP_REQUIRE(grid < (1ll << 31), JSTSP_E_UNSUPPORTED, "hgram grid too large");
    prof_begin(ctx, "gram");
    JSTSP_REQUIRE(!Z2 || zprm, JSTSP_E_NULL, "hgram: Z2 without per-problem scalars");
    if (norm_only && !Z2 && cols >= GRAM_HONLY_MIN_COLS) {
        if (cols % (nsplit * 2 * HBK) == 0)
            hgram_kernel<true, true><<<(unsigned)grid, 256, 0, ctx->stream>>>(Z, sZt, rows, cols, nsplit, amax, Gpart, count, Z2, zprm);
        else
            hgram_kernel<false, true><<<(unsigned)grid, 256, 0, ctx->stream>>>(Z, sZt, rows, cols, nsplit, amax, Gpart, count, Z2, zprm);
    } else
    if (cols % (nsplit * 2 * HBK) == 0)
        hgram_kernel<true><<<(unsigned)grid, 256, 0, ctx->stream>>>(Z, sZt, rows, cols, nsplit, amax, Gpart, count, Z2, zprm);
    else
        hgram_kernel<false><<<(unsigned)grid, 256, 0, ctx->stream>>>(Z, sZt, rows, cols, nsplit, amax, Gpart, count, Z2, zprm);
    prof_end(ctx, "gram");
    JSTSP_HIP(hipGetLastError());
    return 0;
}

int launch_hgram3(jstsp_ctx *ctx, const float2 *X, const float2 *V1, long long sZt, int rows, int cols, int count, int nsplit,
                  const uint32_t *xmax, const uint32_t *vmax, const uint32_t *zmax, const TrialParams *prm, float2 *Gz,
                  float2 *Gx, float2 *Gv)
{
    JSTSP_REQUIRE(rows > 0 && rows <= 64 && cols > 0 && count > 0 && nsplit > 0, JSTSP_E_SHAPE, "hgram3: bad shape");
    const long long grid = (long long)count * nsplit;
    JSTSP_REQUIRE(grid < (1ll << 31), JSTSP_E_UNSUPPORTED, "hgram3 grid too large");
    prof_begin(ctx, "gram");
    const bool nh = cols >= GRAM_HONLY_MIN_COLS;
    if (cols % (nsplit * 2 * HBK) == 0) {
        if (nh) hgram3_kernel<true, true><<<(unsigned)grid, 256, 0, ctx->stream>>>(X, V1, sZt, rows, cols, nsplit, xmax, vmax, zmax, prm, Gz, Gx, Gv, count);
        else hgram3_kernel<true, false><<<(unsigned)grid, 256, 0, ctx->stream>>>(X, V1, sZt, rows, cols, nsplit, xmax, vmax, zmax, prm, Gz, Gx, Gv, count);
    } else {
        if (nh) hgram3_kernel<false, true><<<(unsigned)grid, 256, 0, ctx->stream>>>(X, V1, sZt, rows, cols, nsplit, xmax, vmax, zmax, prm, Gz, Gx, Gv, count);
        else hgram3_kernel<false, false><<<(unsigned)grid, 256, 0, ctx->stream>>>(X, V1, sZt, rows, cols, nsplit, xmax, vmax, zmax, prm, Gz, Gx, Gv, count);
    }
    prof_end(ctx, "gram");
    JSTSP_HIP(hipGetLastError());
    return 0;
}

__global__ __launch_bounds__(256) void herm_fill_kernel(float2 *G, long long sGt, int n)
{
    __shared__ float2 tl[32][33];
    const int nt = (n + 31) / 32;
    const int bi = blockIdx.x % nt, bj = blockIdx.x / nt;
    if (bi < bj) return;
    float2 *g = G + (long long)blockIdx.y * sGt;
    const int tx = threadIdx.x & 31, ty = threadIdx.x >> 5;
    for (int y = ty; y < 32; y += 8) {
        const int r = 32 * bj + tx, c = 32 * bi + y;
        tl[y][tx] = (r < n && c < n) ? g[r + (long long)n * c] : make_float2(0.f, 0.f);
    }
    __syncthreads();
    for (int y = ty; y < 32; y += 8) {
        const int r = 32 * bi + tx, c = 32 * bj + y;
        if (r < n && c < n && r > c) g[r + (long long)n * c] = make_float2(tl[tx][y].x, -tl[tx][y].y);
    }
}

int hermitian_fill_lower(jstsp_ctx *ctx, float2 *G, long long sGt, int n, int count)
{
    const int nt = (n + 31) / 32;
    herm_fill_kernel<<<dim3((unsigned)(nt * nt), count), 256, 0, ctx->stream>>>(G, sGt, n);
    JSTSP_HIP(hipGetLastError());
    return 0;
}

static long long hgemm_grid(HGemmDesc &d, long long tiles, int conc)
{
    d.map_tb = d.map_tt = 0;
    if (d.sPt == 0 && d.batch >= 2 && tiles >= 2) {
        d.map_tb = d.batch < 8 ? d.batch : 8;
        d.map_tt = conc / d.map_tb < 1 ? 1 : conc / d.map_tb;
        if (d.map_tt > tiles) d.map_tt = (int)tiles;
        const long long nb = (long long)((d.batch + d.map_tb - 1) / d.map_tb) * ((tiles + d.map_tt - 1) / d.map_tt);
        return ((nb + 7) / 8) * 8 * d.map_tb * d.map_tt;
    }
    return (long long)((d.batch + 7) / 8) * 8 * tiles;
}

bool hgemm_pair_shape(int m, int n, int batch)
{
    return m == 64 && batch >= 2 && (long long)((batch + 1) / 2) * ((n + 127) / 128) >= 256;
}

int launch_hgemm(jstsp_ctx *ctx, const HGemmDesc &d_in, const char *prof_name)
{
    HGemmDesc d = d_in;
    JSTSP_REQUIRE(d.m > 0 && d.n > 0 && d.k > 0 && d.batch > 0, JSTSP_E_SHAPE, "hgemm: bad shape");
    JSTSP_REQUIRE(d.KS >= 2 * ((d.k + 31) / 32) && d.JT >= 2 * ((d.n + 63) / 64), JSTSP_E_ARG,
                  "hgemm: packed operand smaller than the product");
    const bool wide = !d.Ap && d.epi == EPI_NONE && d.n >= 128 && d.JT * 32 >= ((d.n + 127) / 128) * 128;
    const int tiles_i = (d.m + 63) / 64, tiles_j = wide ? (d.n + 127) / 128 : (d.n + 63) / 64;
    const bool wide_even = wide && (d.k % 32) == 0 && ((d.KS / 2) % 2) == 0 && d.KS == 2 * (d.k / 32);
    JSTSP_REQUIRE((long long)((d.batch + 7) / 8) * 8 * tiles_i * tiles_j < (1ll << 30), JSTSP_E_UNSUPPORTED, "hgemm grid too large");
    if (d.Ap && d.aKS == d.KS && d.sPt == 0 && d.sbmax == 0 && !d.herm_upper && (d.KS % 4) == 0 &&
        hgemm_pair_shape(d.m, d.n, d.batch) && d.JT * 32 >= ((d.n + 127) / 128) * 128) {
        const int npairs = (d.batch + 1) / 2, tj3 = (d.n + 127) / 128;
        d.map_tb = npairs < 4 ? npairs : 4;
        d.map_tt = 32 / d.map_tb < tj3 ? 32 / d.map_tb : tj3;
        const long long nb = (long long)((npairs + d.map_tb - 1) / d.map_tb) * ((tj3 + d.map_tt - 1) / d.map_tt);
        const long long grid3 = ((nb + 7) / 8) * 8 * d.map_tb * d.map_tt;
        JSTSP_REQUIRE(grid3 < (1ll << 31), JSTSP_E_UNSUPPORTED, "hgemm grid too large");
        if (prof_name) prof_begin(ctx, prof_name);
        constexpr int PAIR_LDS = 3 * 2048 * (int)sizeof(uint4);
        auto go = [&](auto kern, int lds) -> int {
            JSTSP_HIP(hipFuncSetAttribute(reinterpret_cast<const void *>(kern), hipFuncAttributeMaxDynamicSharedMemorySize, lds));
            hipLaunchKernelGGL(kern, dim3((unsigned)grid3), dim3(256), lds, ctx->stream, d, tj3, npairs);
            return 0;
        };
        if (d.epi == EPI_UPDATE_C) JSTSP_TRY(go(hgemm_pair_kernel<EPI_UPDATE_C, false>, PAIR_LDS));
        else if (d.k > 1024) JSTSP_TRY(go(hgemm_pair_kernel<EPI_NONE, true>, PAIR_LDS + 65536));
        else JSTSP_TRY(go(hgemm_pair_kernel<EPI_NONE, false>, PAIR_LDS));
        if (prof_name) prof_end(ctx, prof_name);
        JSTSP_HIP(hipGetLastError());
        return 0;
    }
    const int v2_mask = 1;
    const bool pack_ok = d.JT * 32 >= ((d.n + 127) / 128) * 128;
    if (d.m <= 64 && pack_ok && d.Ap && (v2_mask & 1) && d.aKS == d.KS && (d.KS % 4) == 0) {
        const int tj2 = (d.n + 127) / 128;
        const long long grid2 = hgemm_grid(d, tj2, 64);
        if (prof_name) prof_begin(ctx, prof_name);
        if (d.epi == EPI_UPDATE_C)
            hgemm2_kernel<EPI_UPDATE_C, true, 4, 2><<<(unsigned)grid2, 256, 0, ctx->stream>>>(d, tj2);
        else
            hgemm2_kernel<EPI_NONE, true, 4, 2><<<(unsigned)grid2, 256, 0, ctx->stream>>>(d, tj2);
        if (prof_name) prof_end(ctx, prof_name);
        JSTSP_HIP(hipGetLastError());
        return 0;
    }
    if (d.m <= 64 && pack_ok && !d.Ap && (v2_mask & 2) && (d.KS % 4) == 0 && d.epi == EPI_NONE && d.k <= 1024) {
        const int tj2 = (d.n + 127) / 128;
// ... 30 lines not shown
```

jstsp19_amd/csrc/proposed.hip:

```cpp
#include "solver_common.h"
#include <cstdio>
#include <cmath>
#include <cstdlib>
#include <algorithm>

namespace jstsp {

struct ProposedWS {
    float2 *X, *V1, *V2, *C, *Xs, *Y, *ZK, *Zb, *Zb2;
    float *invD;
    float2 *V, *RV, *Res, *RRes, *S, *P1;
    float2 *Tc, *W;
    float2 *GA, *GB;
    TrialParams *prm;
    int32_t *rank;
    double *ce;
    float *lam;
    GramWS gz, gn;
    bool h2 = false;
    HPack Bc, Bs;
    uint32_t *kmax = nullptr, *wmax = nullptr;
    uint32_t *nmax = nullptr, *zmax = nullptr;
    bool h2g = false;
    HPack GBp;
    HPack Wp;
    HPack Kp;
    uint32_t *pmax = nullptr;
};

static int gram3_nsplit(int N, int M, int G2, bool want_ce)
{
    const int chunk = 1024;
    if (!(want_ce && N <= 64 && N <= M && use_hgemm(N, G2, M))) return 0;
    return std::max(1, std::min(32, (M + chunk - 1) / chunk));
}

static size_t proposed_bytes(int N, int M, int Gr, int G2, int batch, int nA, int nB, bool angles,
                             bool want_ce, int Imax)
{
    const size_t nm = (size_t)N * M, g = (size_t)Gr * G2, ng = (size_t)N * G2;
    size_t b = 0;
    b += rnd256(3 * batch * nm * sizeof(float2)) + 6 * rnd256(batch * nm * sizeof(float2));
    b += rnd256(batch * nm * sizeof(float));
    b += 6 * rnd256(batch * g * sizeof(float2));
    b += 2 * rnd256(batch * ng * sizeof(float2));
    b += rnd256((size_t)nA * Gr * Gr * sizeof(float2)) + rnd256((size_t)nB * G2 * G2 * sizeof(float2));
    b += rnd256(batch * sizeof(TrialParams));
    if (angles) b += rnd256(batch * g * sizeof(int32_t));
    b += rnd256((size_t)batch * 3 * Imax * sizeof(double));
    b += rnd256(3 * (size_t)batch * sizeof(float));
    const int ns3 = gram3_nsplit(N, M, G2, want_ce);
    b += GramWS::bytes(N, M, batch, true, ns3);
    if (want_ce) b += GramWS::bytes(N, M, 3 * batch, false, ns3);
    if (use_hgemm(N, G2, M))
        b += hgemm_pack_bytes(M, G2, nB) + hgemm_pack_bytes(G2, M, nB) + 2 * rnd256(8 * batch * sizeof(uint32_t)) +
             hgemm_pack_bytes(G2, N, batch);
    if (use_hgemm(N, G2, M) && nB == 1 && hgemm_pair_shape(N, G2, batch))
        b += rnd256((size_t)batch * 2 * (4 * ((M + 63) / 64)) * 256 * sizeof(uint4));
    if (use_hgemm(Gr, G2, G2)) b += hgemm_pack_bytes(G2, G2, nB) + rnd256(2 * batch * sizeof(uint32_t));
    return b;
}

static int proposed_alloc(Arena &a, ProposedWS &w, int N, int M, int Gr, int G2, int batch, int nA, int nB,
                          bool angles, bool want_ce, int Imax)
{
    const size_t nm = (size_t)N * M, g = (size_t)Gr * G2, ng = (size_t)N * G2;
    w.X = a.get<float2>(3 * batch * nm);
    w.V1 = w.X ? w.X + batch * nm : nullptr;
    w.V2 = w.X ? w.X + 2 * batch * nm : nullptr;
    w.C = a.get<float2>(batch * nm); w.Xs = a.get<float2>(batch * nm); w.Y = a.get<float2>(batch * nm);
    w.ZK = a.get<float2>(batch * nm);
    w.Zb = a.get<float2>(batch * nm);
    w.Zb2 = a.get<float2>(batch * nm);
    w.invD = a.get<float>(batch * nm);
    w.V = a.get<float2>(batch * g); w.RV = a.get<float2>(batch * g); w.Res = a.get<float2>(batch * g);
    w.RRes = a.get<float2>(batch * g); w.S = a.get<float2>(batch * g); w.P1 = a.get<float2>(batch * g);
    w.Tc = a.get<float2>(batch * ng); w.W = a.get<float2>(batch * ng);
    w.GA = a.get<float2>((size_t)nA * Gr * Gr); w.GB = a.get<float2>((size_t)nB * G2 * G2);
    w.prm = a.get<TrialParams>(batch);
    w.rank = angles ? a.get<int32_t>(batch * g) : nullptr;
    w.ce = a.get<double>((size_t)batch * 3 * Imax);
    w.lam = a.get<float>(3 * (size_t)batch);
    JSTSP_REQUIRE(w.X && w.V1 && w.V2 && w.C && w.Xs && w.Y && w.ZK && w.Zb && w.Zb2 && w.invD && w.V && w.RV && w.Res &&
                      w.RRes && w.S && w.P1 && w.Tc && w.W && w.GA && w.GB && w.prm && w.ce && w.lam &&
                      (!angles || w.rank),
                  JSTSP_E_NOMEM, "proposed_algorithm: workspace exhausted");
    const int ns3 = gram3_nsplit(N, M, G2, want_ce);
    JSTSP_TRY(w.gz.alloc(a, N, M, batch, true, ns3));
    if (want_ce) JSTSP_TRY(w.gn.alloc(a, N, M, 3 * batch, false, ns3));
    w.h2 = use_hgemm(N, G2, M);
    if (w.h2) {
        w.kmax = a.get<uint32_t>(16 * (size_t)batch);
        JSTSP_REQUIRE(w.kmax, JSTSP_E_NOMEM, "proposed_algorithm: workspace exhausted");
        w.nmax = w.kmax + batch; w.zmax = w.kmax + 4 * (size_t)batch; w.wmax = w.kmax + 5 * (size_t)batch;
        w.pmax = w.kmax + 6 * (size_t)batch;
        w.Wp.KS = 4 * ((G2 + 63) / 64); w.Wp.JT = 2 * ((N + 63) / 64); w.Wp.count = batch;
        w.Wp.st = (long long)w.Wp.JT * w.Wp.KS * 256;
        w.Wp.data = a.get<uint4>((size_t)batch * w.Wp.st);
        w.Wp.bmax = w.wmax;
        JSTSP_REQUIRE(w.Wp.data, JSTSP_E_NOMEM, "proposed_algorithm: workspace exhausted");
        if (nB == 1 && hgemm_pair_shape(N, G2, batch)) {
            w.Kp.KS = 4 * ((M + 63) / 64); w.Kp.JT = 2; w.Kp.count = batch;
            w.Kp.st = (long long)w.Kp.JT * w.Kp.KS * 256;
            w.Kp.data = a.get<uint4>((size_t)batch * w.Kp.st);
            JSTSP_REQUIRE(w.Kp.data, JSTSP_E_NOMEM, "proposed_algorithm: workspace exhausted");
        }
    }
    w.h2g = use_hgemm(Gr, G2, G2);
    if (w.h2g && !w.pmax) {
        w.pmax = a.get<uint32_t>(2 * (size_t)batch);
        JSTSP_REQUIRE(w.pmax, JSTSP_E_NOMEM, "proposed_algorithm: workspace exhausted");
    }
    return 0;
}

}

using namespace jstsp;

static bool tune_host_pipeline()
{
    load_tuning();
    return tune().host_pipeline != 0;
}

static int proposed_impl(jstsp_ctx *ctx, int N, int M, int Gr, int G2, int batch,
                         const jstsp_c32 *subY_, const float *Omega_,
                         const jstsp_c32 *A_, long long strideA, const jstsp_c32 *B_,
                         long long strideB, int Imax, const double *tau_Y,
                         const double *tau_S, const double *rho, int type,
                         const int32_t *indx_S_, jstsp_c32 *S_out, jstsp_c32 *Y_out,
                         double *ce_out, int memspace, bool allow_fused, std::vector<int> *overflowed, PendingSolve *defer = nullptr)
{
    JSTSP_REQUIRE(ctx, JSTSP_E_NULL, "ctx is NULL");
    JSTSP_REQUIRE(subY_ && Omega_ && A_ && B_ && tau_Y && tau_S && rho && S_out, JSTSP_E_NULL,
                  "proposed_algorithm: NULL array argument");
    JSTSP_REQUIRE(N > 0 && M > 0 && Gr > 0 && G2 > 0 && batch > 0 && Imax >= 0, JSTSP_E_SHAPE,
                  "proposed_algorithm: bad shape N=%d M=%d Gr=%d G2=%d batch=%d Imax=%d", N, M, Gr, G2, batch,
                  Imax);
    JSTSP_REQUIRE(memspace == JSTSP_HOST || memspace == JSTSP_DEVICE, JSTSP_E_ARG, "bad memspace %d",
                  memspace);
    JSTSP_REQUIRE(type == JSTSP_TYPE_APPROXIMATE || type == JSTSP_TYPE_STD, JSTSP_E_ARG, "bad type %d", type);
    JSTSP_REQUIRE(std::min(N, M) <= 2048, JSTSP_E_UNSUPPORTED,
                  "proposed_algorithm: min(N, M) = %d > 2048 (order of the SVT's Gram eigenproblem)",
                  std::min(N, M));
    JSTSP_REQUIRE(strideA == 0 || strideA >= (long long)N * Gr, JSTSP_E_SHAPE, "strideA too small");
    JSTSP_REQUIRE(strideB == 0 || strideB >= (long long)G2 * M, JSTSP_E_SHAPE, "strideB too small");
    const bool approx = type == JSTSP_TYPE_APPROXIMATE;
    JSTSP_REQUIRE(approx || (N >= Gr && M >= G2), JSTSP_E_UNSUPPORTED,
                  "proposed_algorithm 'std': K2 = kron(B.', A) must have full column rank (N >= Gr, M >= G2); the "
                  "under-determined U\\(L\\k) of the reference returns a basic, not least-squares, solution");
    JSTSP_ENTER(ctx);

    const bool angles = indx_S_ != nullptr;
    const bool want_ce = ce_out != nullptr;
    const size_t nm = (size_t)N * M, g = (size_t)Gr * G2, ng = (size_t)N * G2;
    const int nA = strideA ? batch : 1, nB = strideB ? batch : 1;
    const size_t szA = strideA ? (size_t)strideA * (batch - 1) + (size_t)N * Gr : (size_t)N * Gr;
    const size_t szB = strideB ? (size_t)strideB * (batch - 1) + (size_t)G2 * M : (size_t)G2 * M;

    size_t need = proposed_bytes(N, M, Gr, G2, batch, nA, nB, angles, want_ce, std::max(Imax, 1));
    if (!approx)
        need += (pinv_fits(N, Gr) ? rnd256((size_t)nA * Gr * N * sizeof(float2))
                                  : rnd256((size_t)nA * Gr * Gr * sizeof(float2)) + hinv_bytes(Gr, nA)) +
                (pinv_fits(G2, M) ? rnd256((size_t)nB * M * G2 * sizeof(float2))
                                  : rnd256((size_t)nB * G2 * G2 * sizeof(float2)) + hinv_bytes(G2, nB));
    const Tuning &tn = tune();
    const int ftiles = (M % 32 == 0) ? M / 32 : 0;
    const int fparts = tn.fused_parts > 0 ? tn.fused_parts : (ftiles % 4 == 0 ? 4 : (ftiles % 2 == 0 ? 2 : 1));
    const bool want_fused = allow_fused && tn.fused != 0 && approx && Imax > 1 && fused_shape_ok(N, M, G2, fparts);
    if (want_fused) need += fused_bytes(M, G2, nB, batch, fparts);
    need += 1024;
    if (approx)
        need += rnd256((size_t)nA * Gr * Gr * sizeof(float2)) + 2 * rnd256((size_t)nB * (G2 / 2 + 1) * G2 * sizeof(float2));
    const bool host_compact = memspace == JSTSP_HOST && tn.host_compact != 0 && tn.toeplitz != 0 && nB > 1 && G2 >= 32 &&
                              strideB == (long long)G2 * M && (szB * sizeof(float2) >= ((size_t)64 << 20) || tn.host_compact >= 2) &&
                              (long long)G2 * M < (1ll << 31);
    const size_t compact_elems = host_compact ? host_toeplitz_compact_elems(G2, M, nB) : 0;
    if (memspace == JSTSP_HOST) {
        need += rnd256(batch * nm * sizeof(float2)) + rnd256(batch * nm * sizeof(float)) +
                rnd256(szA * sizeof(float2)) + rnd256(szB * sizeof(float2));
        if (angles) need += rnd256(batch * g * sizeof(int32_t));
        need += rnd256(compact_elems * sizeof(float2));
    }
    JSTSP_TRY(ctx->arena.reserve(need));
    ctx->arena.reset();

    const float2 *subY, *A, *B;
    const float *Omega;
    const int32_t *indx_S = nullptr;
    JSTSP_TRY(stage_in(ctx, reinterpret_cast<const float2 *>(subY_), batch * nm, memspace, &subY));
    JSTSP_TRY(stage_in(ctx, Omega_, batch * nm, memspace, &Omega));
    JSTSP_TRY(stage_in(ctx, reinterpret_cast<const float2 *>(A_), szA, memspace, &A));
    int known_gt = ctx->dict_block_hint;
    ctx->dict_block_hint = 0;
    if (host_compact) {
        float2 *Bd = ctx->arena.get<float2>(szB), *Cd = ctx->arena.get<float2>(compact_elems);
        JSTSP_REQUIRE(Bd && Cd, JSTSP_E_NOMEM, "workspace exhausted while staging an input");
        JSTSP_TRY(host_toeplitz_stage(ctx, reinterpret_cast<const float2 *>(B_), G2, M, nB, Bd, Cd, compact_elems, &known_gt));
        if (!known_gt) JSTSP_HIP(hipMemcpyAsync(Bd, B_, szB * sizeof(float2), hipMemcpyHostToDevice, ctx->stream));
        B = Bd;
    } else
    JSTSP_TRY(stage_in(ctx, reinterpret_cast<const float2 *>(B_), szB, memspace, &B));
    if (angles) JSTSP_TRY(stage_in(ctx, indx_S_, batch * g, memspace, &indx_S));
    if (memspace == JSTSP_DEVICE)
        JSTSP_REQUIRE(((uintptr_t)subY % 16 == 0) && ((uintptr_t)Omega % 8 == 0), JSTSP_E_ARG,
                      "device arrays must be 16-byte aligned");

    ProposedWS w;
    JSTSP_TRY(proposed_alloc(ctx->arena, w, N, M, Gr, G2, batch, nA, nB, angles, want_ce, std::max(Imax, 1)));

    {
        std::vector<TrialParams> hp(batch);
        for (int t = 0; t < batch; ++t) hp[t] = make_trial_params(rho[t], tau_Y[t], tau_S[t]);
        JSTSP_TRY(upload(ctx, w.prm, hp.data(), batch * sizeof(TrialParams)));
    }

    hipStream_t st = ctx->stream;
    JSTSP_HIP(hipMemsetAsync(w.X, 0, batch * nm * sizeof(float2), st));
    JSTSP_HIP(hipMemsetAsync(w.V1, 0, batch * nm * sizeof(float2), st));
    JSTSP_HIP(hipMemsetAsync(w.V2, 0, batch * nm * sizeof(float2), st));
    JSTSP_HIP(hipMemsetAsync(w.C, 0, batch * nm * sizeof(float2), st));
    JSTSP_HIP(hipMemsetAsync(w.Xs, 0, batch * nm * sizeof(float2), st));
    JSTSP_HIP(hipMemsetAsync(w.Y, 0, batch * nm * sizeof(float2), st));
    JSTSP_HIP(hipMemsetAsync(w.V, 0, batch * g * sizeof(float2), st));
    JSTSP_HIP(hipMemsetAsync(w.S, 0, batch * g * sizeof(float2), st));
    JSTSP_HIP(hipMemsetAsync(w.ce, 0, (size_t)batch * 3 * std::max(Imax, 1) * sizeof(double), st));
    JSTSP_TRY(launch_inv_d(ctx, (long long)nm, batch, Omega, 2.f, w.prm, w.invD));
    const bool omega_direct = ((uintptr_t)Omega % 16 == 0) && (nm % 4 == 0);
    if (angles) JSTSP_TRY(launch_rank_from_index(ctx, (int)g, batch, indx_S, w.rank));

    const Mat Am{A, strideA, N}, Bm{B, strideB, G2};
    const int toep_env = tn.toeplitz;
    int toep_gt = 0;
    bool toep_probed = false;
    const Mat GAm{w.GA, strideA ? (long long)Gr * Gr : 0, Gr}, GBm{w.GB, strideB ? (long long)G2 * G2 : 0, G2};
    float2 *GAlo = nullptr;
    if (approx) {
        GAlo = ctx->arena.get<float2>((size_t)nA * Gr * Gr);
        JSTSP_REQUIRE(GAlo, JSTSP_E_NOMEM, "proposed_algorithm: workspace exhausted (Gram refinement)");
        JSTSP_TRY(gram_f64(ctx, 'L', A, strideA, N, Gr, nA, w.GA, (long long)Gr * Gr, GAlo));
    } else
    JSTSP_TRY(gemm(ctx, 'C', 'N', Gr, Gr, N, nA, Am, Am, w.GA, (long long)Gr * Gr, Gr));
    if (toep_env != 0 && known_gt && strideB) {
        toep_gt = known_gt;
        toep_probed = true;
    } else
    if (toep_env != 0 && (long long)G2 * M < (1ll << 31) && approx) {
        JSTSP_TRY(fused_probe_toeplitz(ctx, ctx->arena, B, strideB, G2, M, nB, &toep_gt));
        toep_probed = true;
    }
    if (w.h2) {
        JSTSP_TRY(hgemm_pack(ctx, w.Bc, ctx->arena, B, strideB, G2, 1, 1, M, G2, nB, (long long)G2 * M));
    }
    if (approx) {
        if (toep_gt && toep_env >= 2 && M >= G2 / toep_gt) {
            float2 *G0 = ctx->arena.get<float2>((size_t)nB * toep_gt * G2), *G0lo = ctx->arena.get<float2>((size_t)nB * toep_gt * G2);
            JSTSP_REQUIRE(G0 && G0lo, JSTSP_E_NOMEM, "workspace exhausted (G_B block row)");
            GemmDesc dg = make_gemm('N', 'C', toep_gt, G2, M, nB, Bm, Bm, G0, (long long)toep_gt * G2, toep_gt);
            dg.force_m64 = 1; dg.C_lo = G0lo;
            JSTSP_TRY(launch_cgemm(ctx, dg, GEMM_MISC));
            JSTSP_TRY(toeplitz_gram_assemble(ctx, B, strideB, G2, M, toep_gt, nB, G0, G0lo, w.GB, nullptr));
            ctx->last_dict_block = toep_gt;
        } else {
            GemmDesc dg = make_gemm('N', 'C', G2, G2, M, nB, Bm, Bm, w.GB, (long long)G2 * G2, G2);
            dg.force_m64 = 1; dg.herm_upper = 1;
            JSTSP_TRY(launch_cgemm(ctx, dg, GEMM_MISC));
            JSTSP_TRY(hermitian_fill_lower(ctx, w.GB, (long long)G2 * G2, G2, nB));
        }
    } else if (w.h2) {
        {
            HGemmDesc hb{B, strideB, G2, w.Bc.bmax, w.Bc.data, w.Bc.st, w.Bc.bmax, 1, w.Bc.KS, w.Bc.JT, w.GB,
                         (long long)G2 * G2, G2, G2, G2, M, nB, EPI_NONE, nullptr, nullptr, nullptr};
            hb.herm_upper = 1;
            JSTSP_TRY(launch_hgemm(ctx, hb, nullptr));
            JSTSP_TRY(hermitian_fill_lower(ctx, w.GB, (long long)G2 * G2, G2, nB));
        }
    } else
    JSTSP_TRY(gemm(ctx, 'N', 'C', G2, G2, M, nB, Bm, Bm, w.GB, (long long)G2 * G2, G2));

    if (w.h2g && approx)
        JSTSP_TRY(hgemm_pack(ctx, w.GBp, ctx->arena, w.GB, strideB ? (long long)G2 * G2 : 0, 1, G2, 0, G2, G2, nB,
                             (long long)G2 * G2));
    float2 *PA = nullptr, *PB = nullptr;
    if (!approx) {
        JSTSP_TRY(diag_reset(ctx));
        if (pinv_fits(N, Gr)) {
            PA = ctx->arena.get<float2>((size_t)nA * Gr * N);
            JSTSP_REQUIRE(PA, JSTSP_E_NOMEM, "proposed_algorithm 'std': workspace exhausted");
            JSTSP_TRY(launch_pinv(ctx, N, Gr, nA, A, strideA, N, PA, (long long)Gr * N, Gr));
        }
        if (pinv_fits(G2, M)) {
            PB = ctx->arena.get<float2>((size_t)nB * M * G2);
            JSTSP_REQUIRE(PB, JSTSP_E_NOMEM, "proposed_algorithm 'std': workspace exhausted");
            JSTSP_TRY(launch_pinv(ctx, G2, M, nB, B, strideB, G2, PB, (long long)M * G2, M));
        }
        float2 *GAi = PA ? nullptr : ctx->arena.get<float2>((size_t)nA * Gr * Gr);
        float2 *GBi = PB ? nullptr : ctx->arena.get<float2>((size_t)nB * G2 * G2);
        JSTSP_REQUIRE((PA || GAi) && (PB || GBi), JSTSP_E_NOMEM, "proposed_algorithm 'std': workspace exhausted");
        const size_t mark = ctx->arena.off;
        if (!PA) {
            JSTSP_TRY(hermitian_inverse(ctx, Gr, nA, w.GA, GAi));
            ctx->arena.off = mark;
            JSTSP_HIP(hipMemcpyAsync(w.GA, GAi, (size_t)nA * Gr * Gr * sizeof(float2), hipMemcpyDeviceToDevice, st));
        }
        if (!PB) {
            JSTSP_TRY(hermitian_inverse(ctx, G2, nB, w.GB, GBi));
            ctx->arena.off = mark;
            JSTSP_HIP(hipMemcpyAsync(w.GB, GBi, (size_t)nB * G2 * G2 * sizeof(float2), hipMemcpyDeviceToDevice, st));
        }
    }
    const long long snm = (long long)nm, sg = (long long)g, sng = (long long)ng;
    constexpr int rv_refresh = 4;
    auto refresh_at = [](int it) -> bool { return it % rv_refresh == 0; };
    const bool overlap = tn.overlap >= 0 ? tn.overlap != 0 : want_fused;
    uint32_t *const kmax0 = w.kmax;
    JSTSP_TRY(ensure_side_streams(ctx));
    hipStream_t sm = ctx->stream, s1 = overlap ? ctx->side[0] : sm, s2 = overlap ? ctx->side[1] : sm;
    hipEvent_t ev_x = ctx->ev[0], ev_svt = ctx->ev[1], ev_gxv = ctx->ev[2], ev_c = ctx->ev[3], ev_gv2 = ctx->ev[4],
               ev_ce = ctx->ev[5], ev_lxv = ctx->ev[6];
    if (Imax > 0) {
        JSTSP_TRY(launch_form_z(ctx, snm, batch, w.X, w.V1, w.prm, w.Zb));
        JSTSP_TRY(svt_prepare(ctx, w.gz, w.Zb, w.prm, nullptr, true));
    }
    const bool fz = w.gz.left;
    const bool hmax = w.h2 && fz && N <= 64;
    const bool zfly = hmax && want_ce && gram3_nsplit(N, M, G2, want_ce) > 0 && w.gz.nsplit == w.gn.nsplit;
    float2 *Zbuf[2] = {w.Zb, w.Zb2};
    const bool fusedp = want_fused && hmax && (want_ce ? zfly : true);
    const bool fusedy = fusedp;
    FusedWS fw;
    if (fusedp) {
        if (toep_env != 0 && !toep_probed) JSTSP_TRY(fused_probe_toeplitz(ctx, ctx->arena, B, strideB, G2, M, nB, &toep_gt));
        ctx->last_dict_block = toep_gt;
        JSTSP_TRY(fused_alloc(ctx->arena, fw, M, G2, nB, batch, fparts, toep_gt, toep_env >= 2 && fusedy));
        JSTSP_TRY(fused_pack_b(ctx, fw, B, strideB, G2, M, nB, w.Bc.bmax));
        JSTSP_HIP(hipMemsetAsync(fw.ovf, 0, (size_t)batch * sizeof(uint32_t), sm));
    }
    const int fused_kback = tn.fused_kback;
    bool passed = false;
    hipEvent_t ev_q1 = ctx->ev[7], ev_v = ctx->ev[8], ev_rv = ctx->ev[9];
    const bool rv_fused1 = fusedp && tn.grad_fused != 0 && grad_fused_shape(N, Gr, G2);
    const bool rv_early_ok = rv_fused1 && zfly && w.h2g && overlap;
    bool rv_early = false;
    if (want_ce) JSTSP_TRY(lanczos_warm_reset(ctx, w.gn));
    for (int it = 0; it < Imax; ++it) {
        if (want_ce) w.gn.lz.call = it;
        float2 *Zc = fz ? Zbuf[it & 1] : w.Zb, *Zn = fz ? Zbuf[(it + 1) & 1] : w.Zb;
        if (w.h2) {
            const size_t boff = (size_t)(it & 1) * 8 * (size_t)batch;
            w.kmax = kmax0 + boff; w.nmax = w.kmax + batch; w.zmax = w.kmax + 4 * (size_t)batch;
            w.wmax = w.kmax + 5 * (size_t)batch; w.pmax = w.kmax + 6 * (size_t)batch;
            if (!passed) JSTSP_HIP(hipMemsetAsync(w.kmax, 0, 8 * (size_t)batch * sizeof(uint32_t), sm));
        } else if (w.h2g) JSTSP_HIP(hipMemsetAsync(w.pmax, 0, 2 * (size_t)batch * sizeof(uint32_t), sm));
        int apply_no = 0;
        bool next_zeroed = false;
        if (it > 0) JSTSP_HIP(hipStreamWaitEvent(sm, ev_svt, 0));
        if (it > 0 && want_ce) JSTSP_HIP(hipStreamWaitEvent(sm, ev_gxv, 0));
        if (passed) {
        } else if (fz) {
            JSTSP_TRY(launch_eye_minus(ctx, N, batch, w.gz.Q, w.gz.Q));
            GemmDesc dq = make_gemm('N', 'N', N, M, N, batch, Mat{w.gz.Q, (long long)N * N, N}, Mat{Zc, snm, N}, w.Y, snm, N);
            dq.epi = EPI_UPDATE_X; dq.prm = w.prm;
            dq.e_rw0 = w.V1; dq.e_w1 = w.X; dq.e_w2 = w.ZK;
            dq.e_r0 = w.V2; dq.e_r2 = w.Xs; dq.e_r3 = subY; dq.e_f0 = w.invD;
            dq.e_w3 = (it + 1 < Imax && (!zfly || fusedy)) ? Zn : nullptr;
            if (zfly && it > 0) { dq.B = w.X; dq.B2 = w.V1; }
            dq.epi_store_c = (it + 1 == Imax);
            if (w.h2) {
                dq.amax_out = w.kmax;
                if (N <= 64) { dq.amax_x = w.nmax; dq.amax_v1 = w.nmax + batch; dq.amax_z = w.zmax; }
            }
            JSTSP_TRY(launch_cgemm(ctx, dq, GEMM_MISC));
        } else {
            JSTSP_TRY(svt_apply(ctx, w.gz, Zc, w.Y));
            JSTSP_TRY(launch_update_x(ctx, snm, batch, w.X, w.V1, w.V2, w.C, w.Xs, w.Y, subY, w.invD, w.prm, w.ZK));
        }
        JSTSP_HIP(hipEventRecord(ev_x, sm));
        auto issue_s1 = [&](int stage) -> int {
            if (stage != 2) JSTSP_HIP(hipStreamWaitEvent(s1, ev_x, 0));
            StreamScope sc(ctx, s1);
            if (stage != 2 && !fz) JSTSP_TRY(launch_form_z(ctx, snm, batch, w.X, w.V1, w.prm, Zn));
            if (zfly) {
              if (stage != 2) {
                if (fusedp && it > 0) JSTSP_HIP(hipStreamWaitEvent(s1, ev_lxv, 0));
                JSTSP_TRY(launch_hgram3(ctx, w.X, w.V1, snm, N, M, batch, w.gz.nsplit, w.nmax, w.nmax + batch, w.zmax,
                                        w.prm, w.gz.Gpart, w.gn.Gpart, w.gn.Gpart + (size_t)batch * N * N * w.gn.nsplit));
                JSTSP_HIP(hipEventRecord(ev_gxv, s1));
                if (fusedp) {
                    JSTSP_HIP(hipStreamWaitEvent(s2, ev_gxv, 0));
                    StreamScope sc2(ctx, s2);
                    JSTSP_TRY(lmax_from_partials_range(ctx, w.gn, 0, 2 * batch, w.lam, true));
                    JSTSP_HIP(hipEventRecord(ev_lxv, s2));
                }
              }
              if (stage == 1) return 0;
                JSTSP_TRY(svt_prepare(ctx, w.gz, w.X, w.prm, nullptr, true, w.zmax, nullptr, true));
                if (fusedy) JSTSP_TRY(fused_pack_wq(ctx, fw, w.gz.Q, batch));
            } else {
                JSTSP_TRY(svt_prepare(ctx, w.gz, Zn, w.prm, nullptr, true, hmax ? w.zmax : nullptr));
                if (fusedy) JSTSP_TRY(fused_pack_wq(ctx, fw, w.gz.Q, batch));
            }
            JSTSP_HIP(hipEventRecord(ev_svt, s1));
            return 0;
        };
        const bool svt_split = passed && fusedp && zfly && it + 1 < Imax;
        if (it + 1 < Imax) JSTSP_TRY(issue_s1(svt_split ? 1 : 0));
        if (want_ce && !(zfly && it + 1 < Imax)) {
            JSTSP_HIP(hipStreamWaitEvent(s2, ev_x, 0));
            StreamScope sc(ctx, s2);
            JSTSP_TRY(gram_partials_range(ctx, w.gn, w.X, snm, 0, 2 * batch, hmax ? w.nmax : nullptr, nullptr, nullptr, true));
            JSTSP_HIP(hipEventRecord(ev_gxv, s2));
        }
        if (passed) {
            JSTSP_TRY(fused_reduce(ctx, fw, G2, M, batch, w.Tc));
        } else if (PB) {
            JSTSP_TRY(gemm(ctx, 'N', 'N', N, G2, M, batch, Mat{w.ZK, snm, N}, Mat{PB, strideB ? (long long)M * G2 : 0, M},
                           w.Tc, sng, N, 1.f, nullptr, 0, 0, 0.f, GEMM_CORRELATE));
        } else if (w.h2) {
            if (!fz) JSTSP_TRY(hgemm_absmax(ctx, w.ZK, snm, snm, batch, w.kmax));
            HGemmDesc hc{w.ZK, snm, N, w.kmax, w.Bc.data, strideB ? w.Bc.st : 0, w.Bc.bmax, strideB ? 1 : 0, w.Bc.KS,
                         w.Bc.JT, w.Tc, sng, N, N, G2, M, batch, EPI_NONE, nullptr, nullptr, nullptr};
            if (w.Kp.data && !strideB && w.Kp.KS == w.Bc.KS) {
                w.Kp.bmax = w.kmax;
                JSTSP_TRY(hgemm_repack(ctx, w.Kp, w.ZK, snm, N, 1, 0, M, N, w.kmax));
                hc.Ap = w.Kp.data; hc.sApt = w.Kp.st; hc.aKS = w.Kp.KS;
            }
            JSTSP_TRY(launch_hgemm(ctx, hc, "correlate"));
        } else
        JSTSP_TRY(gemm(ctx, 'N', 'C', N, G2, M, batch, Mat{w.ZK, snm, N}, Bm, w.Tc, sng, N, 1.f, nullptr, 0, 0,
                       0.f, GEMM_CORRELATE));
        const long long cnt_ll = std::min<long long>(10 + 5ll * (it + 1), (long long)g);
        const Mat GAl{GAlo, strideA ? (long long)Gr * Gr : 0, Gr};
        auto second_factor = [&](float2 *out, uint32_t *pm, bool exact) -> int {
            if (exact || !w.h2g) {
                GemmDesc dr = make_gemm('N', 'N', Gr, G2, G2, batch, Mat{w.P1, sg, Gr}, GBm, out, sg, Gr);
                dr.force_m64 = exact ? 1 : 0;
                return launch_cgemm(ctx, dr, GEMM_MISC);
            }
            HGemmDesc hg{w.P1, sg, Gr, pm, w.GBp.data, strideB ? w.GBp.st : 0, w.GBp.bmax, strideB ? 1 : 0,
                         w.GBp.KS, w.GBp.JT, out, sg, Gr, Gr, G2, G2, batch, EPI_NONE, nullptr, nullptr, nullptr};
            return launch_hgemm(ctx, hg, nullptr);
        };
        auto apply_R = [&](const float2 *Xin, float2 *out, bool exact) -> int {
            uint32_t *pm = w.pmax ? w.pmax + (size_t)(apply_no++ & 1) * batch : nullptr;
            if (exact && rv_fused1) {
                JSTSP_TRY(launch_grad_refresh_p1(ctx, Xin, w.GA, GAlo, strideA ? (long long)Gr * Gr : 0, w.P1, G2, batch));
                return second_factor(out, pm, exact);
            }
            if (exact) JSTSP_TRY(gemm(ctx, 'N', 'N', Gr, G2, Gr, batch, GAl, Mat{Xin, sg, Gr}, w.P1, sg, Gr));
            GemmDesc dp = make_gemm('N', 'N', Gr, G2, Gr, batch, GAm, Mat{Xin, sg, Gr}, w.P1, sg, Gr, 1.f, exact ? w.P1 : nullptr, sg,
                                    Gr, exact ? 1.f : 0.f);
            dp.amax_out = w.h2g ? pm : nullptr;
            JSTSP_TRY(launch_cgemm(ctx, dp, GEMM_MISC));
            return second_factor(out, pm, exact);
        };
        if (approx) {
            const bool refreshed = refresh_at(it);
            if (refreshed && rv_early) {
                JSTSP_HIP(hipStreamWaitEvent(sm, ev_rv, 0));
                rv_early = false;
            } else if (refreshed) JSTSP_TRY(apply_R(w.V, w.RV, true));
            if (svt_split && tn.grad_fused != 0 && w.h2g && grad_fused_shape(N, Gr, G2)) {
                uint32_t *pm = w.pmax + (size_t)(apply_no++ & 1) * batch;
                JSTSP_TRY(launch_grad_res_p1(ctx, A, strideA, w.Tc, w.RV, w.Res, w.GA, strideA ? (long long)Gr * Gr : 0, w.P1, pm,
                                             G2, batch));
                JSTSP_TRY(second_factor(w.RRes, pm, false));
            } else {
            GemmDesc dres = make_gemm('C', 'N', Gr, G2, N, batch, Am, Mat{w.Tc, sng, N}, w.Res, sg, Gr, 1.f, w.RV, sg, Gr, -1.f);
            JSTSP_TRY(launch_cgemm(ctx, dres, GEMM_MISC));
            JSTSP_TRY(apply_R(w.Res, w.RRes, false));
            }
            if (svt_split) {
                JSTSP_HIP(hipEventRecord(ev_q1, sm));
                JSTSP_HIP(hipStreamWaitEvent(s1, ev_q1, 0));
                JSTSP_TRY(issue_s1(2));
            }
            const bool early_next = rv_early_ok && it + 1 < Imax && refresh_at(it + 1);
            uint32_t *const nx_zero = (fusedp && tn.grad_fused != 0 && it + 1 < Imax) ? kmax0 + (size_t)((it + 1) & 1) * 8 * (size_t)batch : nullptr;
            if (nx_zero && it > 0 && want_ce) JSTSP_HIP(hipStreamWaitEvent(sm, ev_gv2, 0));
            next_zeroed = nx_zero != nullptr;
            JSTSP_TRY(launch_step_v(ctx, (int)g, batch, w.Res, w.RRes, w.V, w.S, w.rank, (int)cnt_ll, w.prm, w.ce,
                                    Imax, it, early_next ? nullptr : w.RV, svt_split, nx_zero));
            if (early_next) {
                JSTSP_HIP(hipEventRecord(ev_v, sm));
                JSTSP_HIP(hipStreamWaitEvent(s2, ev_v, 0));
                StreamScope sc(ctx, s2);
                JSTSP_TRY(launch_grad_refresh_p1(ctx, w.V, w.GA, GAlo, strideA ? (long long)Gr * Gr : 0, w.P1, G2, batch));
                JSTSP_TRY(second_factor(w.RV, nullptr, true));
                JSTSP_HIP(hipEventRecord(ev_rv, s2));
                rv_early = true;
            }
        } else {
            float2 *left = PB ? w.V : w.P1;
            if (PA)
                JSTSP_TRY(gemm(ctx, 'N', 'N', Gr, G2, N, batch, Mat{PA, strideA ? (long long)Gr * N : 0, Gr},
                               Mat{w.Tc, sng, N}, left, sg, Gr));
            else {
                JSTSP_TRY(gemm(ctx, 'C', 'N', Gr, G2, N, batch, Am, Mat{w.Tc, sng, N}, w.Res, sg, Gr));
                JSTSP_TRY(gemm(ctx, 'N', 'N', Gr, G2, Gr, batch, GAm, Mat{w.Res, sg, Gr}, left, sg, Gr));
            }
            if (!PB) JSTSP_TRY(gemm(ctx, 'N', 'N', Gr, G2, G2, batch, Mat{w.P1, sg, Gr}, GBm, w.V, sg, Gr));
            JSTSP_TRY(launch_soft(ctx, (int)g, batch, w.V, w.S, w.rank, (int)cnt_ll, w.prm));
        }
        if (fusedp && !want_ce && it + 1 == Imax) break;
        if (w.h2) {
            GemmDesc dw = make_gemm('N', 'N', N, G2, Gr, batch, Am, Mat{w.S, sg, Gr}, w.W, sng, N);
            dw.amax_out = w.wmax;
            JSTSP_TRY(launch_cgemm(ctx, dw, GEMM_MISC));
        } else
        JSTSP_TRY(gemm(ctx, 'N', 'N', N, G2, Gr, batch, Am, Mat{w.S, sg, Gr}, w.W, sng, N));
        if (it > 0 && want_ce) JSTSP_HIP(hipStreamWaitEvent(sm, ev_gv2, 0));
        passed = false;
        if (fusedp && it + 1 < Imax) {
            uint32_t *nx = kmax0 + (size_t)((it + 1) & 1) * 8 * (size_t)batch;
            if (!next_zeroed) JSTSP_HIP(hipMemsetAsync(nx, 0, 8 * (size_t)batch * sizeof(uint32_t), sm));
            JSTSP_TRY(fused_pack_as(ctx, fw, w.W, sng, G2, M, batch, w.wmax));
            JSTSP_HIP(hipStreamWaitEvent(sm, ev_svt, 0));
            FusedDesc fd{fw.Bf, strideB ? fw.sBf : 0, w.Bc.bmax, strideB ? 1 : 0, fw.ASp, fw.sAS, w.wmax, w.kmax,
                         w.X, w.V1, w.V2, subY, w.Y, omega_direct ? Omega : w.invD, snm, w.prm, fw.Ppart,
                         nx, nx + batch, nx + 2 * (size_t)batch, nx + 4 * (size_t)batch, w.nmax + 2 * (size_t)batch, fw.ovf,
                         M, G2, batch, fparts,
                         fusedy ? fw.Wqp : nullptr, Zbuf[(it + 1) & 1], w.zmax,
                         (fw.v2 && zfly) ? nullptr : Zbuf[it & 1],
                         (fusedy && it + 2 == Imax) ? w.Y : nullptr, fused_kback,
                         fw.Ec, strideB ? fw.sEc : 0, fw.gt ? 31 - __builtin_clz((unsigned)fw.gt) : 0, fw.ecols, fw.ehalo,
                         fw.v2, fw.XsD, fw.Kf, omega_direct ? 1 : 0};
            JSTSP_TRY(launch_fused_pass(ctx, fd));
            passed = true;
        } else
        if (w.h2) {
            JSTSP_TRY(hgemm_repack(ctx, w.Wp, w.W, sng, N, 1, 0, G2, N, w.wmax));
            if (!w.Bs.data)
                JSTSP_TRY(hgemm_pack(ctx, w.Bs, ctx->arena, B, strideB, 1, G2, 0, G2, M, nB, (long long)G2 * M, w.Bc.bmax));
            HGemmDesc hs{w.W, sng, N, w.wmax, w.Bs.data, strideB ? w.Bs.st : 0, w.Bs.bmax, strideB ? 1 : 0, w.Bs.KS,
                         w.Bs.JT, w.Xs, snm, N, N, M, G2, batch, fz ? EPI_UPDATE_C : EPI_NONE, w.prm, w.X, w.V2,
                         hmax ? w.nmax + 2 * (size_t)batch : nullptr, w.Wp.data, w.Wp.st, w.Wp.KS};
            JSTSP_TRY(launch_hgemm(ctx, hs, "synthesize"));
            if (!fz) JSTSP_TRY(launch_update_c(ctx, snm, batch, w.X, w.Xs, w.V2, w.C, w.prm));
        } else if (fz) {
            GemmDesc ds = make_gemm('N', 'N', N, M, G2, batch, Mat{w.W, sng, N}, Bm, w.Xs, snm, N);
            ds.epi = EPI_UPDATE_C; ds.prm = w.prm;
            ds.e_r0 = w.X; ds.e_rw0 = w.V2;
            JSTSP_TRY(launch_cgemm(ctx, ds, GEMM_SYNTH));
        } else {
            JSTSP_TRY(gemm(ctx, 'N', 'N', N, M, G2, batch, Mat{w.W, sng, N}, Bm, w.Xs, snm, N, 1.f, nullptr, 0, 0,
                           0.f, GEMM_SYNTH));
            JSTSP_TRY(launch_update_c(ctx, snm, batch, w.X, w.Xs, w.V2, w.C, w.prm));
        }
        if (want_ce) {
            JSTSP_HIP(hipEventRecord(ev_c, sm));
            JSTSP_HIP(hipStreamWaitEvent(s2, ev_c, 0));
            if (zfly) JSTSP_HIP(hipStreamWaitEvent(s2, ev_gxv, 0));
            StreamScope sc(ctx, s2);
            JSTSP_TRY(gram_partials_range(ctx, w.gn, w.X, snm, 2 * batch, batch, hmax ? w.nmax : nullptr, nullptr, nullptr, true));
            JSTSP_HIP(hipEventRecord(ev_gv2, s2));
            if (fusedp && zfly && it + 1 < Imax) JSTSP_TRY(lmax_from_partials_range(ctx, w.gn, 2 * batch, batch, w.lam, true));
            else JSTSP_TRY(lmax_from_partials(ctx, w.gn, w.lam, true));
            JSTSP_TRY(launch_ce_ratio(ctx, batch, w.lam + batch, w.lam + 2 * batch, w.lam, w.ce, Imax, it));
            JSTSP_HIP(hipEventRecord(ev_ce, s2));
        }
    }
    if (want_ce && Imax > 0) JSTSP_HIP(hipStreamWaitEvent(sm, ev_ce, 0));
    if (defer) {
        defer->active = true; defer->fused = fusedp; defer->want_ce = want_ce && Imax > 0; defer->batch = batch; defer->g = g; defer->nm = nm;
        defer->Imax = Imax; defer->dS = w.S; defer->dY = w.Y; defer->dce = w.ce; defer->ovf = fusedp ? fw.ovf : nullptr;
        return 0;
    }

    JSTSP_TRY(stage_out(ctx, reinterpret_cast<float2 *>(S_out), w.S, batch * g, memspace));
    JSTSP_TRY(stage_out(ctx, reinterpret_cast<float2 *>(Y_out), w.Y, batch * nm, memspace));
    if (want_ce && Imax > 0) JSTSP_TRY(stage_out(ctx, ce_out, w.ce, (size_t)batch * 3 * Imax, memspace));
    if (fusedp && overflowed) {
        std::vector<uint32_t> flags(batch);
        JSTSP_HIP(hipMemcpyAsync(flags.data(), fw.ovf, (size_t)batch * sizeof(uint32_t), hipMemcpyDeviceToHost, st));
        JSTSP_HIP(hipStreamSynchronize(st));
        for (int t = 0; t < batch; ++t)
            if (flags[t]) overflowed->push_back(t);
    }
    if (memspace == JSTSP_HOST) {
        JSTSP_HIP(hipStreamSynchronize(st));
        if (!approx) JSTSP_TRY(diag_check_host(ctx, "proposed_algorithm 'std'"));
    }
    return 0;
}

static int resolve_overflowed(jstsp_ctx *ctx, const std::vector<int> &ovf, int N, int M, int Gr, int G2, const jstsp_c32 *subY,
                              const float *Omega, const jstsp_c32 *A, long long strideA, const jstsp_c32 *B, long long strideB,
                              int Imax, const double *tau_Y, const double *tau_S, const double *rho, int type,
                              const int32_t *indx_S, jstsp_c32 *S_out, jstsp_c32 *Y_out, double *ce_out, int memspace, int *count)
{
    const size_t nm = (size_t)N * M, g = (size_t)Gr * G2;
    for (size_t i = 0; i < ovf.size();) {
        size_t j = i + 1;
        while (j < ovf.size() && ovf[j] == ovf[j - 1] + 1) ++j;
        const int t0 = ovf[i], cnt = (int)(j - i);
        JSTSP_TRY(proposed_impl(ctx, N, M, Gr, G2, cnt, subY + t0 * nm, Omega + t0 * nm, A + (size_t)t0 * strideA, strideA,
                                B + (size_t)t0 * strideB, strideB, Imax, tau_Y + t0, tau_S + t0, rho + t0, type,
                                indx_S ? indx_S + t0 * g : nullptr, S_out + t0 * g, Y_out ? Y_out + t0 * nm : nullptr,
                                ce_out ? ce_out + (size_t)t0 * 3 * Imax : nullptr, memspace, false, nullptr));
        *count += cnt;
        i = j;
    }
    return 0;
}

static int proposed_finish(jstsp_ctx *ctx, const PendingSolve &p, jstsp_c32 *S_out, jstsp_c32 *Y_out, double *ce_out, std::vector<int> *ovf)
{
    JSTSP_ENTER(ctx);
    JSTSP_TRY(stage_out(ctx, reinterpret_cast<float2 *>(S_out), p.dS, p.batch * p.g, JSTSP_HOST));
    JSTSP_TRY(stage_out(ctx, reinterpret_cast<float2 *>(Y_out), p.dY, p.batch * p.nm, JSTSP_HOST));
    if (p.want_ce) JSTSP_TRY(stage_out(ctx, ce_out, p.dce, (size_t)p.batch * 3 * p.Imax, JSTSP_HOST));
    std::vector<uint32_t> flags(p.ovf ? p.batch : 0);
    if (p.ovf) JSTSP_HIP(hipMemcpyAsync(flags.data(), p.ovf, (size_t)p.batch * sizeof(uint32_t), hipMemcpyDeviceToHost, ctx->stream));
    JSTSP_HIP(hipStreamSynchronize(ctx->stream));
    for (int t = 0; t < (int)flags.size(); ++t)
        if (flags[t]) ovf->push_back(t);
    return 0;
}

extern "C" int jstsp_proposed_algorithm_c32(jstsp_ctx *ctx, int N, int M, int Gr, int G2, int batch,
                                            const jstsp_c32 *subY, const float *Omega,
                                            const jstsp_c32 *A, long long strideA, const jstsp_c32 *B,
                                            long long strideB, int Imax, const double *tau_Y,
                                            const double *tau_S, const double *rho, int type,
                                            const int32_t *indx_S, jstsp_c32 *S_out, jstsp_c32 *Y_out,
                                            double *ce_out, int memspace)
{
    std::vector<int> ovf;
    if (ctx) { ctx->fused_fallbacks = 0; ctx->last_dict_block = 0; }
    const size_t nm = (size_t)N * M, g = (size_t)Gr * G2;
    const size_t in_bytes = (size_t)batch * (nm * 12 + (strideB ? (size_t)G2 * M * 8 : 0));
    const bool pipeline = ctx && memspace == JSTSP_HOST && type == JSTSP_TYPE_APPROXIMATE && batch >= 128 && Imax > 1 && Y_out &&
                          in_bytes >= ((size_t)256 << 20) && subY && Omega && A && B && tau_Y && tau_S && rho && S_out &&
                          tune_host_pipeline();
    if (pipeline) {
        if (!ctx->helper) JSTSP_TRY(jstsp_create(ctx->device, &ctx->helper));
        jstsp_ctx *cx[2] = {ctx, ctx->helper};
        const int h = ((batch / 2 + 7) / 8) * 8, cnt[2] = {h, batch - h}, t0[2] = {0, h};
        PendingSolve pend[2];
        auto drained = [&](int rc) {
            if (rc) for (int k = 0; k < 2; ++k) { DeviceScope ds(cx[k]->device); (void)hipStreamSynchronize(cx[k]->stream); }
            return rc;
        };
#define JSTSP_TRY_PIPE(expr) do { int rc_ = drained(expr); if (rc_ != 0) return rc_; } while (0)
        for (int k = 0; k < 2; ++k) {
            cx[k]->fused_fallbacks = 0; cx[k]->last_dict_block = 0;
            JSTSP_TRY_PIPE(proposed_impl(cx[k], N, M, Gr, G2, cnt[k], subY + t0[k] * nm, Omega + t0[k] * nm, A + (size_t)t0[k] * strideA, strideA,
                                    B + (size_t)t0[k] * strideB, strideB, Imax, tau_Y + t0[k], tau_S + t0[k], rho + t0[k], type,
                                    indx_S ? indx_S + t0[k] * g : nullptr, S_out + t0[k] * g, Y_out + t0[k] * nm,
                                    ce_out ? ce_out + (size_t)t0[k] * 3 * Imax : nullptr, JSTSP_HOST, true, nullptr, &pend[k]));
        }
        int fallbacks = 0;
        for (int k = 0; k < 2; ++k) {
            std::vector<int> o;
            JSTSP_TRY_PIPE(proposed_finish(cx[k], pend[k], S_out + t0[k] * g, Y_out + t0[k] * nm, ce_out ? ce_out + (size_t)t0[k] * 3 * Imax : nullptr, &o));
            JSTSP_TRY_PIPE(resolve_overflowed(cx[k], o, N, M, Gr, G2, subY + t0[k] * nm, Omega + t0[k] * nm, A + (size_t)t0[k] * strideA, strideA,
                                         B + (size_t)t0[k] * strideB, strideB, Imax, tau_Y + t0[k], tau_S + t0[k], rho + t0[k], type,
                                         indx_S ? indx_S + t0[k] * g : nullptr, S_out + t0[k] * g, Y_out + t0[k] * nm,
                                         ce_out ? ce_out + (size_t)t0[k] * 3 * Imax : nullptr, JSTSP_HOST, &fallbacks));
        }
#undef JSTSP_TRY_PIPE
        ctx->fused_fallbacks = fallbacks;
        ctx->last_dict_block = (cx[0]->last_dict_block == cx[1]->last_dict_block) ? cx[0]->last_dict_block : 0;
        return 0;
    }
    JSTSP_TRY(proposed_impl(ctx, N, M, Gr, G2, batch, subY, Omega, A, strideA, B, strideB, Imax, tau_Y, tau_S, rho, type,
                            indx_S, S_out, Y_out, ce_out, memspace, true, &ovf));
    int fallbacks = 0;
    JSTSP_TRY(resolve_overflowed(ctx, ovf, N, M, Gr, G2, subY, Omega, A, strideA, B, strideB, Imax, tau_Y, tau_S, rho, type, indx_S, S_out,
                                 Y_out, ce_out, memspace, &fallbacks));
    ctx->fused_fallbacks += fallbacks;
    return 0;
}

struct jstsp_pending {
    int N, M, Gr, G2, batch, Imax, type;
    const jstsp_c32 *subY, *A, *B;
    const float *Omega;
    long long strideA, strideB;
    const int32_t *indx_S;
    jstsp_c32 *S_out, *Y_out;
    double *ce_out;
    std::vector<double> tau_Y, tau_S, rho;
    uint32_t *flags = nullptr;
    hipEvent_t done = nullptr;
};

extern "C" int jstsp_proposed_algorithm_begin_c32(jstsp_ctx *ctx, int N, int M, int Gr, int G2, int batch, const jstsp_c32 *subY,
                                                  const float *Omega, const jstsp_c32 *A, long long strideA, const jstsp_c32 *B,
                                                  long long strideB, int Imax, const double *tau_Y, const double *tau_S,
                                                  const double *rho, int type, const int32_t *indx_S, jstsp_c32 *S_out,
                                                  jstsp_c32 *Y_out, double *ce_out, jstsp_pending **pending)
{
    JSTSP_REQUIRE(ctx && pending, JSTSP_E_NULL, "proposed_algorithm_begin: NULL context or handle pointer");
    *pending = nullptr;
    ctx->fused_fallbacks = 0; ctx->last_dict_block = 0;
    PendingSolve ps;
    JSTSP_TRY(proposed_impl(ctx, N, M, Gr, G2, batch, subY, Omega, A, strideA, B, strideB, Imax, tau_Y, tau_S, rho, type, indx_S, S_out,
                            Y_out, ce_out, JSTSP_DEVICE, true, nullptr, &ps));
    JSTSP_ENTER(ctx);
    JSTSP_TRY(stage_out(ctx, reinterpret_cast<float2 *>(S_out), ps.dS, ps.batch * ps.g, JSTSP_DEVICE));
    JSTSP_TRY(stage_out(ctx, reinterpret_cast<float2 *>(Y_out), ps.dY, ps.batch * ps.nm, JSTSP_DEVICE));
    if (ps.want_ce) JSTSP_TRY(stage_out(ctx, ce_out, ps.dce, (size_t)ps.batch * 3 * ps.Imax, JSTSP_DEVICE));
    jstsp_pending *p = new (std::nothrow) jstsp_pending();
    JSTSP_REQUIRE(p, JSTSP_E_NOMEM, "proposed_algorithm_begin: out of host memory");
    p->N = N; p->M = M; p->Gr = Gr; p->G2 = G2; p->batch = batch; p->Imax = Imax; p->type = type;
    p->subY = subY; p->A = A; p->B = B; p->Omega = Omega; p->strideA = strideA; p->strideB = strideB; p->indx_S = indx_S;
    p->S_out = S_out; p->Y_out = Y_out; p->ce_out = ce_out;
    p->tau_Y.assign(tau_Y, tau_Y + batch); p->tau_S.assign(tau_S, tau_S + batch); p->rho.assign(rho, rho + batch);
    hipError_t e = hipSuccess;
    if (ps.ovf) {
        e = hipHostMalloc((void **)&p->flags, (size_t)batch * sizeof(uint32_t), hipHostMallocDefault);
        if (e == hipSuccess) e = hipMemcpyAsync(p->flags, ps.ovf, (size_t)batch * sizeof(uint32_t), hipMemcpyDeviceToHost, ctx->stream);
    }
    if (e == hipSuccess) e = hipEventCreateWithFlags(&p->done, hipEventDisableTiming);
    if (e == hipSuccess) e = hipEventRecord(p->done, ctx->stream);
    const int rc = (int)e;
    if (rc) {
        (void)hipStreamSynchronize(ctx->stream);
        if (p->flags) (void)hipHostFree(p->flags);
        if (p->done) (void)hipEventDestroy(p->done);
        delete p;
        set_error("proposed_algorithm_begin: could not set up the completion record: %s", hipGetErrorString(e));
// ... 74 lines not shown
```

jstsp19_amd/csrc/solver_common.h:

```cpp
#pragma once
#include "common.h"
#include <vector>

namespace jstsp {

struct Mat {
    const float2 *p; long long st; int ld;
};

int gemm(jstsp_ctx *ctx, char opA, char opB, int m, int n, int k, int batch, Mat A, Mat B, float2 *C,
         long long sCt, int ldc, float alpha = 1.f, const float2 *D = nullptr, long long sDt = 0,
         int ldd = 0, float beta = 0.f, int tag = GEMM_MISC, int splitk = 1, long long sCsplit = 0);

int gram_f64(jstsp_ctx *ctx, char side, const float2 *X, long long sXt, int rows, int cols, int count, float2 *G, long long sGt,
             float2 *Glo = nullptr);

bool grad_head_shape_ok(int N, int Gr, int G2);
int launch_grad_head(jstsp_ctx *ctx, int G2, int batch, const float2 *P, long long sPt, long long sPp, int parts, const float2 *Kf,
                     const float2 *Bdl, long long sBdl, const float2 *A, long long sA, const float2 *GA, long long sGA,
                     const float2 *RV, float2 *Tc, float2 *Res, float2 *P1, uint32_t *pmax);

GemmDesc make_gemm(char opA, char opB, int m, int n, int k, int batch, Mat A, Mat B, float2 *C, long long sCt,
                   int ldc, float alpha = 1.f, const float2 *D = nullptr, long long sDt = 0, int ldd = 0,
                   float beta = 0.f, int splitk = 1, long long sCsplit = 0);

struct GramWS {
    int rows = 0, cols = 0, n = 0, nsplit = 1, batch = 0;
    bool left = true;
    float2 *Gpart = nullptr;
    float2 *Q = nullptr;
    float2 *Vg = nullptr;
    float2 *Uwarm = nullptr;
    float2 *Twarm = nullptr;
    mutable int warm = 0;
    float eig_stop = 0.f;
    mutable LanczosWarm lz;
    static size_t bytes(int rows, int cols, int batch, bool need_q, int force_nsplit = 0);
    int alloc(Arena &a, int rows, int cols, int batch, bool need_q, int force_nsplit = 0);
};

int gram_partials(jstsp_ctx *ctx, const GramWS &w, const float2 *Z, long long sZt);
int svt_batched(jstsp_ctx *ctx, const GramWS &w, const float2 *Z, const TrialParams *prm,
                const float *tau, float2 *Y, bool sequence = false);
int svt_prepare(jstsp_ctx *ctx, const GramWS &w, const float2 *Z, const TrialParams *prm, const float *tau,
                bool sequence, const uint32_t *amax = nullptr, const float2 *Z2 = nullptr,
                bool gram_done = false);
int svt_apply(jstsp_ctx *ctx, const GramWS &w, const float2 *Z, float2 *Y);
int gram_partials_range(jstsp_ctx *ctx, const GramWS &w, const float2 *Z, long long sZt, int t0, int count,
                        const uint32_t *amax = nullptr, const float2 *Z2 = nullptr,
                        const TrialParams *zprm = nullptr, bool norm_only = false);
int lanczos_warm_reset(jstsp_ctx *ctx, const GramWS &w);
int lmax_from_partials(jstsp_ctx *ctx, const GramWS &w, float *lam, bool lanczos = false);
int lmax_from_partials_range(jstsp_ctx *ctx, const GramWS &w, int first, int count, float *lam, bool lanczos);
int ensure_side_streams(jstsp_ctx *ctx);
int ensure_bj_resources(jstsp_ctx *ctx);
bool ensure_cu_streams(jstsp_ctx *ctx);
struct StreamScope {
    jstsp_ctx *c; hipStream_t saved;
    StreamScope(jstsp_ctx *ctx, hipStream_t s) : c(ctx), saved(ctx->stream) { c->stream = s; }
    ~StreamScope() { c->stream = saved; }
};
int sigma_max_sq(jstsp_ctx *ctx, const GramWS &w, const float2 *Z, float *lam, bool lanczos = false);

size_t hinv_bytes(int n, int count);
int hermitian_inverse(jstsp_ctx *ctx, int n, int count, const float2 *G, float2 *Ginv);

bool pinv_fits(int rows, int cols);
int launch_pinv(jstsp_ctx *ctx, int rows, int cols, int count, const float2 *A, long long sAt, int lda, float2 *P,
                long long sPt, int ldp, float *rcond_out = nullptr);
int ensure_diag(jstsp_ctx *ctx);
int diag_reset(jstsp_ctx *ctx);
int diag_check_host(jstsp_ctx *ctx, const char *what);

struct PendingSolve {
    bool active = false, fused = false, want_ce = false;
    int batch = 0;
    size_t g = 0, nm = 0;
    int Imax = 0;
    const float2 *dS = nullptr, *dY = nullptr;
    const double *dce = nullptr;
    const uint32_t *ovf = nullptr;
};
int proposed_enqueue_device(jstsp_ctx *ctx, int N, int M, int Gr, int G2, int batch, const jstsp_c32 *subY, const float *Omega,
                            const jstsp_c32 *A, long long strideA, const jstsp_c32 *B, long long strideB, int Imax,
                            const double *tau_Y, const double *tau_S, const double *rho, int type, const int32_t *indx_S,
                            bool want_ce, PendingSolve *out);
int proposed_pending_flags(jstsp_ctx *ctx, const PendingSolve &p, std::vector<int> *ovf);
int proposed_resolve_device(jstsp_ctx *ctx, int N, int M, int Gr, int G2, int batch, const jstsp_c32 *subY, const float *Omega,
                            const jstsp_c32 *A, long long strideA, const jstsp_c32 *B, long long strideB, int Imax,
                            const double *tau_Y, const double *tau_S, const double *rho, int type, const int32_t *indx_S,
                            jstsp_c32 *S_dev, jstsp_c32 *Y_dev, double *ce_dev);

int upload(jstsp_ctx *ctx, void *dst, const void *src, size_t bytes);

template <class T> int stage_in(jstsp_ctx *ctx, const T *src, size_t n, int memspace, const T **out)
{
    if (memspace == JSTSP_DEVICE) { *out = src; return 0; }
    T *d = ctx->arena.get<T>(n);
    JSTSP_REQUIRE(d, JSTSP_E_NOMEM, "workspace exhausted while staging an input");
    JSTSP_HIP(hipMemcpyAsync(d, src, n * sizeof(T), hipMemcpyHostToDevice, ctx->stream));
    *out = d;
    return 0;
}
template <class T> int stage_out(jstsp_ctx *ctx, T *dst, const T *dev, size_t n, int memspace)
{
    if (!dst) return 0;
    JSTSP_HIP(hipMemcpyAsync(dst, dev, n * sizeof(T),
                             memspace == JSTSP_DEVICE ? hipMemcpyDeviceToDevice : hipMemcpyDeviceToHost,
                             ctx->stream));
    return 0;
}
inline size_t rnd256(size_t b) { return (b + 255) & ~size_t(255); }

template <class T>
int host_toeplitz_stage(jstsp_ctx *ctx, const T *Bh, int G2, int M, int nB, float2 *Bdev, float2 *Cdev, size_t cdev_elems, int *gt_out);
size_t host_toeplitz_compact_elems(int G2, int M, int nB);

struct FusedWS {
    uint4 *Bf = nullptr; long long sBf = 0;
    uint4 *ASp = nullptr; long long sAS = 0;
    float2 *Ppart = nullptr;
    uint32_t *ovf = nullptr;
    uint4 *Wqp = nullptr;
    int parts = 0;
    uint4 *Ec = nullptr; long long sEc = 0;
    int gt = 0, ecols = 0, ehalo = 0;
    int v2 = 0;
    const float2 *Bsrc = nullptr; long long sBsrc = 0;
    float2 *Bdl = nullptr; long long sBdl = 0;
    float2 *XsD = nullptr, *Kf = nullptr;
};
struct FusedDesc {
    const uint4 *Bf; long long sBf;
    const uint32_t *bmax; int sbmax;
    const uint4 *ASp; long long sAS;
    const uint32_t *wmax;
    const uint32_t *kmax_prev;
    float2 *X, *V1, *V2;
    const float2 *subY, *Y; const float *invD;
    long long snm;
    const TrialParams *prm;
    float2 *Ppart;
    uint32_t *kmax_out, *xmax, *v1max, *zmax, *v2max, *ovf;
    int M, G2, batch, parts;
    const uint4 *Wqp; const float2 *Zin; const uint32_t *zmax_in; float2 *Zout, *Yout;
    int kback;
    const uint4 *Ec; long long sEc; int gsh, ecols, ehalo;
    int v2; const float2 *XsD; float2 *Kf;
    int inv_is_omega;
};
bool fused_shape_ok(int N, int M, int G2, int parts);
size_t fused_bytes(int M, int G2, int nB, int batch, int parts);
int fused_probe_toeplitz(jstsp_ctx *ctx, Arena &ar, const float2 *B, long long sBt, int G2, int M, int nB, int *gt);
int toeplitz_gram_assemble(jstsp_ctx *ctx, const float2 *B, long long sBt, int G2, int M, int gt, int nB, const float2 *G0,
                           const float2 *G0lo, float2 *G, float2 *Glo);
int fused_alloc(Arena &ar, FusedWS &f, int M, int G2, int nB, int batch, int parts, int gt, int v2);
int fused_pack_b(jstsp_ctx *ctx, FusedWS &f, const float2 *B, long long sBt, int G2, int M, int nB, const uint32_t *bmax);
int fused_pack_as(jstsp_ctx *ctx, const FusedWS &f, const float2 *W, long long sWt, int G2, int M, int batch, const uint32_t *wmax);
int launch_fused_pass(jstsp_ctx *ctx, const FusedDesc &d);
int fused_reduce(jstsp_ctx *ctx, const FusedWS &f, int G2, int M, int batch, float2 *Tc);
int fused_pack_wq(jstsp_ctx *ctx, const FusedWS &f, const float2 *Q, int batch);

bool grad_fused_shape(int N, int Gr, int G2);
int launch_grad_res_p1(jstsp_ctx *ctx, const float2 *A, long long sAt, const float2 *Tc, const float2 *RV, float2 *Res,
                       const float2 *GA, long long sGAt, float2 *P1, uint32_t *pmax, int G2, int batch);
int launch_grad_refresh_p1(jstsp_ctx *ctx, const float2 *V, const float2 *GA, const float2 *GAlo, long long sGAt, float2 *P1, int G2,
                           int batch);

}
```

Before: 848.0 channel-estimates/s.

## Streamline solver setup: skip zero-state work, fuse probe absmax, Toeplitz-aware packing

Setup work that only handles the known all-zero initial state is removed. Memsets of X, V1, C, Xs and Y are skipped, the first z formation becomes a memset, and the first x-update GEMM is replaced by an elementwise first_x kernel that also produces the abs-max scales. The Toeplitz probe now computes the dictionary abs-max while it verifies, so a separate absmax pass is avoided. The dictionary packers read through the block-Toeplitz map to get better locality. The final Y is written straight into the device output, which drops a copy. Aliasing checks guard the direct write, and correctness depends on the zero-init assumptions holding.

Result: no change. 855.0 channel-estimates/s (median of 6 runs) (+0.8%).

```diff
diff --git a/jstsp19_amd/csrc/admm.hip b/jstsp19_amd/csrc/admm.hip
--- a/jstsp19_amd/csrc/admm.hip
+++ b/jstsp19_amd/csrc/admm.hip
@@ -51,6 +51,73 @@
                 Z[base + j] = make_float2(admm_z(p, x.x, v.x), admm_z(p, x.y, v.y));
             }
         }
+    }
+}
+
+__device__ __forceinline__ void first_x_one(const TrialParams &p, float z0, float sy, float id, float &x, float &k, float &v1, float &zn)
+{
+    x = admm_x(p, z0, z0, sy, z0, z0, id);
+    k = admm_k(p, x, z0);
+    v1 = admm_v1(p, z0, z0, x);
+    zn = admm_z(p, x, v1);
+}
+
+__global__ __launch_bounds__(256) void first_x_kernel(long long nm, const float2 *subY, const float *invD, const TrialParams *prm,
+                                                      float z0, float2 *X, float2 *K, float2 *V1, float2 *Zn, float2 *Y,
+                                                      uint32_t *kmax, uint32_t *xmax, uint32_t *v1max, uint32_t *zmax)
+{
+    const int t = blockIdx.y;
+    const TrialParams p = prm[t];
+    const long long base = (long long)t * nm;
+    const long long stride = (long long)gridDim.x * 256 * 2;
+    const bool vec = (nm & 1) == 0;
+    float mk = 0.f, mx = 0.f, mv = 0.f, mz = 0.f;
+    for (long long i = ((long long)blockIdx.x * 256 + threadIdx.x) * 2; i < nm; i += stride) {
+        if (vec && i + 1 < nm) {
+            const c2 sy = ld2(subY, base + i);
+            const float2 id = *reinterpret_cast<const float2 *>(invD + base + i);
+            c2 x, k, v1, zn;
+            first_x_one(p, z0, sy.a.x, id.x, x.a.x, k.a.x, v1.a.x, zn.a.x);
+            first_x_one(p, z0, sy.a.y, id.x, x.a.y, k.a.y, v1.a.y, zn.a.y);
+            first_x_one(p, z0, sy.b.x, id.y, x.b.x, k.b.x, v1.b.x, zn.b.x);
+            first_x_one(p, z0, sy.b.y, id.y, x.b.y, k.b.y, v1.b.y, zn.b.y);
+            st2(X, base + i, x); st2(K, base + i, k); st2(V1, base + i, v1);
+            if (Zn) st2(Zn, base + i, zn);
+            if (Y) { c2 y; y.a = y.b = make_float2(z0, z0); st2(Y, base + i, y); }
+            mk = fmaxf(fmaxf(mk, fmaxf(fabsf(k.a.x), fabsf(k.a.y))), fmaxf(fabsf(k.b.x), fabsf(k.b.y)));
+            mx = fmaxf(fmaxf(mx, fmaxf(fabsf(x.a.x), fabsf(x.a.y))), fmaxf(fabsf(x.b.x), fabsf(x.b.y)));
+            mv = fmaxf(fmaxf(mv, fmaxf(fabsf(v1.a.x), fabsf(v1.a.y))), fmaxf(fabsf(v1.b.x), fabsf(v1.b.y)));
+            mz = fmaxf(fmaxf(mz, fmaxf(fabsf(zn.a.x), fabsf(zn.a.y))), fmaxf(fabsf(zn.b.x), fabsf(zn.b.y)));
+        } else {
+            for (long long j = i; j < nm && j < i + 2; ++j) {
+                const float2 sy = subY[base + j];
+                const float id = invD[base + j];
+                float2 x, k, v1, zn;
+                first_x_one(p, z0, sy.x, id, x.x, k.x, v1.x, zn.x);
+                first_x_one(p, z0, sy.y, id, x.y, k.y, v1.y, zn.y);
+                X[base + j] = x; K[base + j] = k; V1[base + j] = v1;
+                if (Zn) Zn[base + j] = zn;
+                if (Y) Y[base + j] = make_float2(z0, z0);
+                mk = fmaxf(mk, fmaxf(fabsf(k.x), fabsf(k.y)));
+                mx = fmaxf(mx, fmaxf(fabsf(x.x), fabsf(x.y)));
+                mv = fmaxf(mv, fmaxf(fabsf(v1.x), fabsf(v1.y)));
+                mz = fmaxf(mz, fmaxf(fabsf(zn.x), fabsf(zn.y)));
+            }
+        }
+    }
+    if (!kmax && !xmax) return;
+#pragma unroll
+    for (int o = 32; o > 0; o >>= 1) {
+        mk = fmaxf(mk, __shfl_xor(mk, o)); mx = fmaxf(mx, __shfl_xor(mx, o));
+        mv = fmaxf(mv, __shfl_xor(mv, o)); mz = fmaxf(mz, __shfl_xor(mz, o));
+    }
+    __shared__ float sh[4][4];
+    if ((threadIdx.x & 63) == 0) { const int w = threadIdx.x >> 6; sh[0][w] = mk; sh[1][w] = mx; sh[2][w] = mv; sh[3][w] = mz; }
+    __syncthreads();
+    if (threadIdx.x < 4) {
+        uint32_t *const dst = threadIdx.x == 0 ? kmax : threadIdx.x == 1 ? xmax : threadIdx.x == 2 ? v1max : zmax;
+        const float *r = sh[threadIdx.x];
+        if (dst) atomicMax(&dst[t], __float_as_uint(fmaxf(fmaxf(r[0], r[1]), fmaxf(r[2], r[3]))));
     }
 }
 
@@ -286,6 +353,14 @@
     JSTSP_HIP(hipGetLastError());
     return 0;
 }
+int launch_first_x(jstsp_ctx *ctx, long long nm, int batch, const float2 *subY, const float *invD, const TrialParams *prm, float2 *X,
+                   float2 *K, float2 *V1, float2 *Zn, float2 *Y, uint32_t *kmax, uint32_t *xmax, uint32_t *v1max, uint32_t *zmax)
+{
+    hipLaunchKernelGGL(first_x_kernel, ew_grid(nm, batch), dim3(256), 0, ctx->stream, nm, subY, invD, prm, 0.f, X, K, V1, Zn, Y, kmax,
+                       xmax, v1max, zmax);
+    JSTSP_HIP(hipGetLastError());
+    return 0;
+}
 int launch_update_x(jstsp_ctx *ctx, long long nm, int batch, float2 *X, float2 *V1, const float2 *V2,
                     const float2 *C, const float2 *Xs, const float2 *Y, const float2 *subY,
                     const float *invD, const TrialParams *prm, float2 *K)
diff --git a/jstsp19_amd/csrc/common.h b/jstsp19_amd/csrc/common.h
--- a/jstsp19_amd/csrc/common.h
+++ b/jstsp19_amd/csrc/common.h
@@ -271,7 +271,7 @@
 bool hgemm_pair_shape(int m, int n, int batch);
 int hgemm_absmax(jstsp_ctx *ctx, const float2 *X, long long n, long long sXt, int count, uint32_t *amax);
 int hgemm_pack(jstsp_ctx *ctx, HPack &p, Arena &ar, const float2 *B, long long sBt, long long sBk, long long sBj,
-               int conj, int Kd, int J, int count, long long n_contig, const uint32_t *bmax_known = nullptr);
+               int conj, int Kd, int J, int count, long long n_contig, const uint32_t *bmax_known = nullptr, int toep_gt = 0);
 int hgemm_repack(jstsp_ctx *ctx, const HPack &p, const float2 *B, long long sBt, long long sBk, long long sBj, int conj,
                  int Kd, int J, const uint32_t *bmax);
 int launch_hgemm(jstsp_ctx *ctx, const HGemmDesc &d, const char *prof_name = nullptr);
@@ -304,6 +304,8 @@
 
 int launch_form_z(jstsp_ctx *ctx, long long nm, int batch, const float2 *X, const float2 *V1,
                   const TrialParams *prm, float2 *Z);
+int launch_first_x(jstsp_ctx *ctx, long long nm, int batch, const float2 *subY, const float *invD, const TrialParams *prm, float2 *X,
+                   float2 *K, float2 *V1, float2 *Zn, float2 *Y, uint32_t *kmax, uint32_t *xmax, uint32_t *v1max, uint32_t *zmax);
 int launch_update_x(jstsp_ctx *ctx, long long nm, int batch, float2 *X, float2 *V1,
                     const float2 *V2, const float2 *C, const float2 *Xs, const float2 *Y,
                     const float2 *subY, const float *invD, const TrialParams *prm, float2 *K);
diff --git a/jstsp19_amd/csrc/fused.hip b/jstsp19_amd/csrc/fused.hip
--- a/jstsp19_amd/csrc/fused.hip
+++ b/jstsp19_amd/csrc/fused.hip
@@ -124,6 +124,41 @@
 #pragma unroll
     for (int o = 32; o > 0; o >>= 1) bad |= __shfl_xor(bad, o);
     if ((threadIdx.x & 63) == 0 && (bad & ~__atomic_load_n(mism, __ATOMIC_RELAXED))) atomicOr(mism, bad);
+}
+
+__global__ __launch_bounds__(256) void toeplitz_verify_max_kernel(const float2 *B, long long sBt, int G2, int M, int c, uint32_t *mism,
+                                                                  uint32_t *bmax)
+{
+    const uint32_t qpc = (uint32_t)G2 >> 2, nq = qpc * (uint32_t)M;
+    const uint4 *b = reinterpret_cast<const uint4 *>(reinterpret_cast<const uint2 *>(B) + (long long)blockIdx.y * sBt);
+    const int gt = 16 << c;
+    uint32_t bad = 0;
+    float mx = 0.f;
+    for (uint32_t q = blockIdx.x * 256u + threadIdx.x; q < nq; q += gridDim.x * 256u) {
+        const int m = (int)(q / qpc), g = 4 * (int)(q - (uint32_t)m * qpc);
+        const int ld = g >> (4 + c);
+        const uint32_t e = (uint32_t)g + (uint32_t)G2 * (uint32_t)m;
+        const uint4 x0 = b[e >> 1], x1 = b[(e >> 1) + 1];
+        mx = fmaxf(mx, fmaxf(fmaxf(fmaxf(fabsf(__uint_as_float(x0.x)), fabsf(__uint_as_float(x0.y))),
+                                   fmaxf(fabsf(__uint_as_float(x0.z)), fabsf(__uint_as_float(x0.w)))),
+                             fmaxf(fmaxf(fabsf(__uint_as_float(x1.x)), fabsf(__uint_as_float(x1.y))),
+                                   fmaxf(fabsf(__uint_as_float(x1.z)), fabsf(__uint_as_float(x1.w))))));
+        if (ld >= 1 && m >= ld) {
+            const uint32_t f = e - (uint32_t)gt - (uint32_t)G2;
+            const uint4 y0 = b[f >> 1], y1 = b[(f >> 1) + 1];
+            if (x0.x != y0.x || x0.y != y0.y || x0.z != y0.z || x0.w != y0.w || x1.x != y1.x || x1.y != y1.y || x1.z != y1.z ||
+                x1.w != y1.w)
+                bad = 1u << c;
+        }
+    }
+#pragma unroll
+    for (int o = 32; o > 0; o >>= 1) { bad |= __shfl_xor(bad, o); mx = fmaxf(mx, __shfl_xor(mx, o)); }
+    if ((threadIdx.x & 63) == 0 && (bad & ~__atomic_load_n(mism, __ATOMIC_RELAXED))) atomicOr(mism, bad);
+    __shared__ float sm[4];
+    if ((threadIdx.x & 63) == 0) sm[threadIdx.x >> 6] = mx;
+    __syncthreads();
+    if (threadIdx.x == 0)
+        atomicMax(&bmax[blockIdx.y], __float_as_uint(fmaxf(fmaxf(sm[0], sm[1]), fmaxf(sm[2], sm[3]))));
 }
 
 __global__ __launch_bounds__(256) void pack_e_kernel(const float2 *B, long long sBt, int G2, int M, int gt, int ecols, int ehalo,
@@ -966,7 +1001,8 @@
            rnd256((size_t)nB * G2 * 8 * sizeof(float2)) + 512;
 }
 
-int fused_probe_toeplitz(jstsp_ctx *ctx, Arena &ar, const float2 *B, long long sBt, int G2, int M, int nB, int *gt)
+int fused_probe_toeplitz(jstsp_ctx *ctx, Arena &ar, const float2 *B, long long sBt, int G2, int M, int nB, int *gt, uint32_t *bmax,
+                         bool *bmax_valid)
 {
     *gt = 0;
     uint32_t *flag = ar.get<uint32_t>(1);
@@ -978,7 +1014,13 @@
     const unsigned nblk = (unsigned)(((long long)G2 * M + 255) / 256);
     for (int step = 0; step < (nB > 1 ? 2 : 1) && cand; ++step) {
         JSTSP_HIP(hipMemsetAsync(flag, 0, sizeof(uint32_t), ctx->stream));
-        if (step && sBt % 2 == 0)
+        if (step && sBt % 2 == 0 && bmax) {
+            JSTSP_HIP(hipMemsetAsync(bmax, 0, (size_t)nB * sizeof(uint32_t), ctx->stream));
+            const unsigned nb4 = (nblk + 3) / 4, per = std::max(32u, (2048u + (unsigned)nB - 1) / (unsigned)nB);
+            hipLaunchKernelGGL(toeplitz_verify_max_kernel, dim3(std::min(nb4, per), nB), dim3(256), 0, ctx->stream, B, sBt, G2, M,
+                               31 - __builtin_clz(cand), flag, bmax);
+            *bmax_valid = true;
+        } else if (step && sBt % 2 == 0)
             hipLaunchKernelGGL(toeplitz_verify_kernel, dim3((nblk + 3) / 4, nB), dim3(256), 0, ctx->stream, B, sBt, G2, M,
                                31 - __builtin_clz(cand), flag);
         else
diff --git a/jstsp19_amd/csrc/hgemm.hip b/jstsp19_amd/csrc/hgemm.hip
--- a/jstsp19_amd/csrc/hgemm.hip
+++ b/jstsp19_amd/csrc/hgemm.hip
@@ -71,6 +71,84 @@
         _Float16 h, l;
         split2(x.x * s, h, l); rh[v] = h; rl[v] = l;
         split2(x.y * sg, h, l); ih[v] = h; il[v] = l;
+    }
+    uint4 *o = out + (((long long)t * JT + jt) * KS + ks) * 256 + lane;
+    o[0] = *reinterpret_cast<uint4 *>(&rh);
+    o[64] = *reinterpret_cast<uint4 *>(&rl);
+    o[128] = *reinterpret_cast<uint4 *>(&ih);
+    o[192] = *reinterpret_cast<uint4 *>(&il);
+}
+
+__global__ __launch_bounds__(256) void pack_b_toep_kernel(const float2 *B, long long sBt, int G2, int gsh, int kis_m, int conj, int Kd,
+                                                          int J, int KS, int JT, const uint32_t *bmax, uint4 *out)
+{
+    const int t = blockIdx.y;
+    uint32_t bx = blockIdx.x;
+    if (!kis_m && (gridDim.x & 63u) == 0) bx = (bx & ~63u) | ((bx & 7u) << 3) | ((bx >> 3) & 7u);
+    const long long idx = (long long)bx * 256 + threadIdx.x;
+    if (idx >= (long long)JT * KS * 64) return;
+    const int lane = (int)(idx & 63);
+    const long long blk = idx >> 6;
+    const int ks = (int)(blk % KS), jt = (int)(blk / KS);
+    const int j = jt * 32 + (lane & 31), k0 = ks * 16 + 8 * (lane >> 5);
+    const float s = ldexpf(1.f, scale_exp(bmax[t]));
+    const float sg = conj ? -s : s;
+    const float2 *b = B + (long long)t * sBt;
+    half8 rh, rl, ih, il;
+#pragma unroll
+    for (int v = 0; v < 8; ++v) {
+        float2 x = make_float2(0.f, 0.f);
+        if (j < J && k0 + v < Kd) {
+            int g = kis_m ? j : k0 + v, m = kis_m ? k0 + v : j;
+            const int ld = g >> gsh;
+            if (m >= ld) { g -= ld << gsh; m -= ld; }
+            x = b[(long long)g + (long long)m * G2];
+        }
+        _Float16 h, l;
+        split2(x.x * s, h, l); rh[v] = h; rl[v] = l;
+        split2(x.y * sg, h, l); ih[v] = h; il[v] = l;
+    }
+    uint4 *o = out + (((long long)t * JT + jt) * KS + ks) * 256 + lane;
+    o[0] = *reinterpret_cast<uint4 *>(&rh);
+    o[64] = *reinterpret_cast<uint4 *>(&rl);
+    o[128] = *reinterpret_cast<uint4 *>(&ih);
+    o[192] = *reinterpret_cast<uint4 *>(&il);
+}
+
+__global__ __launch_bounds__(256) void pack_bs_toep_kernel(const float2 *B, long long sBt, int G2, int M, int gsh, int KS, int JT,
+                                                           const uint32_t *bmax, uint4 *out)
+{
+    __shared__ float2 tile[32][65];
+    const int t = blockIdx.y;
+    uint32_t bx = blockIdx.x;
+    if ((gridDim.x & 63u) == 0) bx = (bx & ~63u) | ((bx & 7u) << 3) | ((bx >> 3) & 7u);
+    const long long blk0 = (long long)bx * 4;
+    if (blk0 >= (long long)JT * KS) return;
+    const int ks0 = (int)(blk0 % KS), jt = (int)(blk0 / KS);
+    const float2 *b = B + (long long)t * sBt;
+#pragma unroll
+    for (int i = 0; i < 8; ++i) {
+        const int e = threadIdx.x + 256 * i, r = e & 63, c = e >> 6;
+        int g = ks0 * 16 + r, m = jt * 32 + c;
+        float2 x = make_float2(0.f, 0.f);
+        if (g < G2 && m < M) {
+            const int ld = g >> gsh;
+            if (m >= ld) { g -= ld << gsh; m -= ld; }
+            x = b[(long long)g + (long long)m * G2];
+        }
+        tile[c][r] = x;
+    }
+    __syncthreads();
+    const int lane = threadIdx.x & 63, w = threadIdx.x >> 6;
+    const int ks = ks0 + w, r0 = 16 * w + 8 * (lane >> 5), c = lane & 31;
+    const float s = ldexpf(1.f, scale_exp(bmax[t]));
+    half8 rh, rl, ih, il;
+#pragma unroll
+    for (int v = 0; v < 8; ++v) {
+        const float2 x = tile[c][r0 + v];
+        _Float16 h, l;
+        split2(x.x * s, h, l); rh[v] = h; rl[v] = l;
+        split2(x.y * s, h, l); ih[v] = h; il[v] = l;
     }
     uint4 *o = out + (((long long)t * JT + jt) * KS + ks) * 256 + lane;
     o[0] = *reinterpret_cast<uint4 *>(&rh);
@@ -1067,8 +1145,10 @@
 }
 
 int hgemm_pack(jstsp_ctx *ctx, HPack &p, Arena &ar, const float2 *B, long long sBt, long long sBk, long long sBj,
-               int conj, int Kd, int J, int count, long long n_contig, const uint32_t *bmax_known)
-{
+               int conj, int Kd, int J, int count, long long n_contig, const uint32_t *bmax_known, int toep_gt)
+{
+    JSTSP_REQUIRE(toep_gt == 0 || ((toep_gt & (toep_gt - 1)) == 0 && ((sBk == 1 && sBj == Kd) || (sBj == 1 && sBk == J))), JSTSP_E_ARG,
+                  "hgemm_pack: the block-Toeplitz source map needs a column-major dictionary");
     p.KS = 4 * ((Kd + 63) / 64);
     p.JT = 4 * ((J + 127) / 128);
     p.count = count;
@@ -1079,6 +1159,13 @@
     if (bmax_known) JSTSP_HIP(hipMemcpyAsync(p.bmax, bmax_known, (size_t)count * sizeof(uint32_t), hipMemcpyDeviceToDevice, ctx->stream));
     else JSTSP_TRY(hgemm_absmax(ctx, B, n_contig, sBt, count, p.bmax));
     const long long slots = (long long)p.JT * p.KS * 64;
+    if (toep_gt && sBj != 1 && !conj)
+        pack_bs_toep_kernel<<<dim3((unsigned)((slots + 255) / 256), count), 256, 0, ctx->stream>>>(
+            B, sBt, Kd, J, 31 - __builtin_clz((unsigned)toep_gt), p.KS, p.JT, p.bmax, p.data);
+    else if (toep_gt)
+        pack_b_toep_kernel<<<dim3((unsigned)((slots + 255) / 256), count), 256, 0, ctx->stream>>>(
+            B, sBt, sBj == 1 ? J : Kd, 31 - __builtin_clz((unsigned)toep_gt), sBj == 1 ? 1 : 0, conj, Kd, J, p.KS, p.JT, p.bmax, p.data);
+    else
     pack_b_kernel<<<dim3((unsigned)((slots + 255) / 256), count), 256, 0, ctx->stream>>>(B, sBt, sBk, sBj, conj, Kd, J,
                                                                                          p.KS, p.JT, p.bmax, p.data);
     JSTSP_HIP(hipGetLastError());
diff --git a/jstsp19_amd/csrc/proposed.hip b/jstsp19_amd/csrc/proposed.hip
--- a/jstsp19_amd/csrc/proposed.hip
+++ b/jstsp19_amd/csrc/proposed.hip
@@ -170,7 +170,8 @@
     const int fparts = tn.fused_parts > 0 ? tn.fused_parts : (ftiles % 4 == 0 ? 4 : (ftiles % 2 == 0 ? 2 : 1));
     const bool want_fused = allow_fused && tn.fused != 0 && approx && Imax > 1 && fused_shape_ok(N, M, G2, fparts);
     if (want_fused) need += fused_bytes(M, G2, nB, batch, fparts);
-    need += 1024;
+    need += 1024 + rnd256((size_t)nB * sizeof(uint32_t));
+    const bool lean_setup = tn.fused != 2;
     if (approx)
         need += rnd256((size_t)nA * Gr * Gr * sizeof(float2)) + 2 * rnd256((size_t)nB * (G2 / 2 + 1) * G2 * sizeof(float2));
     const bool host_compact = memspace == JSTSP_HOST && tn.host_compact != 0 && tn.toeplitz != 0 && nB > 1 && G2 >= 32 &&
@@ -217,12 +218,15 @@
     }
 
     hipStream_t st = ctx->stream;
-    JSTSP_HIP(hipMemsetAsync(w.X, 0, batch * nm * sizeof(float2), st));
-    JSTSP_HIP(hipMemsetAsync(w.V1, 0, batch * nm * sizeof(float2), st));
+    const bool epi_path = w.gz.left;
+    if (!lean_setup || !epi_path) {
+        JSTSP_HIP(hipMemsetAsync(w.X, 0, batch * nm * sizeof(float2), st));
+        JSTSP_HIP(hipMemsetAsync(w.V1, 0, batch * nm * sizeof(float2), st));
+    }
     JSTSP_HIP(hipMemsetAsync(w.V2, 0, batch * nm * sizeof(float2), st));
-    JSTSP_HIP(hipMemsetAsync(w.C, 0, batch * nm * sizeof(float2), st));
-    JSTSP_HIP(hipMemsetAsync(w.Xs, 0, batch * nm * sizeof(float2), st));
-    JSTSP_HIP(hipMemsetAsync(w.Y, 0, batch * nm * sizeof(float2), st));
+    if (!lean_setup || !epi_path) JSTSP_HIP(hipMemsetAsync(w.C, 0, batch * nm * sizeof(float2), st));
+    if (!lean_setup || !epi_path) JSTSP_HIP(hipMemsetAsync(w.Xs, 0, batch * nm * sizeof(float2), st));
+    if (!lean_setup || !epi_path || Imax == 0) JSTSP_HIP(hipMemsetAsync(w.Y, 0, batch * nm * sizeof(float2), st));
     JSTSP_HIP(hipMemsetAsync(w.V, 0, batch * g * sizeof(float2), st));
     JSTSP_HIP(hipMemsetAsync(w.S, 0, batch * g * sizeof(float2), st));
     JSTSP_HIP(hipMemsetAsync(w.ce, 0, (size_t)batch * 3 * std::max(Imax, 1) * sizeof(double), st));
@@ -234,6 +238,8 @@
     const int toep_env = tn.toeplitz;
     int toep_gt = 0;
     bool toep_probed = false;
+    const uint32_t *probe_bmax = nullptr;
+    bool probe_bmax_valid = false;
     const Mat GAm{w.GA, strideA ? (long long)Gr * Gr : 0, Gr}, GBm{w.GB, strideB ? (long long)G2 * G2 : 0, G2};
     float2 *GAlo = nullptr;
     if (approx) {
@@ -247,11 +253,14 @@
         toep_probed = true;
     } else
     if (toep_env != 0 && (long long)G2 * M < (1ll << 31) && approx) {
-        JSTSP_TRY(fused_probe_toeplitz(ctx, ctx->arena, B, strideB, G2, M, nB, &toep_gt));
+        uint32_t *pb = (lean_setup && w.h2 && nB > 1) ? ctx->arena.get<uint32_t>(nB) : nullptr;
+        JSTSP_TRY(fused_probe_toeplitz(ctx, ctx->arena, B, strideB, G2, M, nB, &toep_gt, pb, &probe_bmax_valid));
+        if (probe_bmax_valid) probe_bmax = pb;
         toep_probed = true;
     }
+    const int pack_gt = lean_setup ? toep_gt : 0;
     if (w.h2) {
-        JSTSP_TRY(hgemm_pack(ctx, w.Bc, ctx->arena, B, strideB, G2, 1, 1, M, G2, nB, (long long)G2 * M));
+        JSTSP_TRY(hgemm_pack(ctx, w.Bc, ctx->arena, B, strideB, G2, 1, 1, M, G2, nB, (long long)G2 * M, probe_bmax, pack_gt));
     }
     if (approx) {
         if (toep_gt && toep_env >= 2 && M >= G2 / toep_gt) {
@@ -320,6 +329,8 @@
     hipEvent_t ev_x = ctx->ev[0], ev_svt = ctx->ev[1], ev_gxv = ctx->ev[2], ev_c = ctx->ev[3], ev_gv2 = ctx->ev[4],
                ev_ce = ctx->ev[5], ev_lxv = ctx->ev[6];
     if (Imax > 0) {
+        if (lean_setup && epi_path) JSTSP_HIP(hipMemsetAsync(w.Zb, 0, batch * nm * sizeof(float2), sm));
+        else
         JSTSP_TRY(launch_form_z(ctx, snm, batch, w.X, w.V1, w.prm, w.Zb));
         JSTSP_TRY(svt_prepare(ctx, w.gz, w.Zb, w.prm, nullptr, true));
     }
@@ -328,6 +339,15 @@
     const bool zfly = hmax && want_ce && gram3_nsplit(N, M, G2, want_ce) > 0 && w.gz.nsplit == w.gn.nsplit;
     float2 *Zbuf[2] = {w.Zb, w.Zb2};
     const bool fusedp = want_fused && hmax && (want_ce ? zfly : true);
+    auto overlaps = [&](const void *p, size_t bytes) {
+        const uintptr_t a0 = (uintptr_t)Y_out, a1 = a0 + batch * nm * sizeof(float2), b0 = (uintptr_t)p;
+        return b0 < a1 && a0 < b0 + bytes;
+    };
+    const bool y_direct = lean_setup && memspace == JSTSP_DEVICE && !defer && Y_out && fz && Imax > 0 && ((uintptr_t)Y_out % 16 == 0) &&
+                          nm % 2 == 0 && !overlaps(subY, batch * nm * sizeof(float2)) && !overlaps(Omega, batch * nm * sizeof(float)) &&
+                          !overlaps(A, szA * sizeof(float2)) && !overlaps(B, szB * sizeof(float2)) &&
+                          !overlaps(S_out, batch * g * sizeof(float2)) && !(indx_S && overlaps(indx_S, batch * g * sizeof(int32_t)));
+    float2 *const Yfinal = y_direct ? reinterpret_cast<float2 *>(Y_out) : w.Y;
     const bool fusedy = fusedp;
     FusedWS fw;
     if (fusedp) {
@@ -358,9 +378,16 @@
         if (it > 0) JSTSP_HIP(hipStreamWaitEvent(sm, ev_svt, 0));
         if (it > 0 && want_ce) JSTSP_HIP(hipStreamWaitEvent(sm, ev_gxv, 0));
         if (passed) {
+        } else if (fz && it == 0 && lean_setup) {
+            JSTSP_TRY(launch_eye_minus(ctx, N, batch, w.gz.Q, w.gz.Q));
+            JSTSP_TRY(launch_first_x(ctx, snm, batch, subY, w.invD, w.prm, w.X, w.ZK, w.V1,
+                                     (it + 1 < Imax && (!zfly || fusedy)) ? Zn : nullptr, it + 1 == Imax ? Yfinal : nullptr,
+                                     w.h2 ? w.kmax : nullptr, (w.h2 && N <= 64) ? w.nmax : nullptr,
+                                     (w.h2 && N <= 64) ? w.nmax + batch : nullptr, (w.h2 && N <= 64) ? w.zmax : nullptr));
         } else if (fz) {
             JSTSP_TRY(launch_eye_minus(ctx, N, batch, w.gz.Q, w.gz.Q));
-            GemmDesc dq = make_gemm('N', 'N', N, M, N, batch, Mat{w.gz.Q, (long long)N * N, N}, Mat{Zc, snm, N}, w.Y, snm, N);
+            GemmDesc dq = make_gemm('N', 'N', N, M, N, batch, Mat{w.gz.Q, (long long)N * N, N}, Mat{Zc, snm, N},
+                                   it + 1 == Imax ? Yfinal : w.Y, snm, N);
             dq.epi = EPI_UPDATE_X; dq.prm = w.prm;
             dq.e_rw0 = w.V1; dq.e_w1 = w.X; dq.e_w2 = w.ZK;
             dq.e_r0 = w.V2; dq.e_r2 = w.Xs; dq.e_r3 = subY; dq.e_f0 = w.invD;
@@ -523,7 +550,7 @@
                          M, G2, batch, fparts,
                          fusedy ? fw.Wqp : nullptr, Zbuf[(it + 1) & 1], w.zmax,
                          (fw.v2 && zfly) ? nullptr : Zbuf[it & 1],
-                         (fusedy && it + 2 == Imax) ? w.Y : nullptr, fused_kback,
+                         (fusedy && it + 2 == Imax) ? Yfinal : nullptr, fused_kback,
                          fw.Ec, strideB ? fw.sEc : 0, fw.gt ? 31 - __builtin_clz((unsigned)fw.gt) : 0, fw.ecols, fw.ehalo,
                          fw.v2, fw.XsD, fw.Kf, omega_direct ? 1 : 0};
             JSTSP_TRY(launch_fused_pass(ctx, fd));
@@ -532,7 +559,7 @@
         if (w.h2) {
             JSTSP_TRY(hgemm_repack(ctx, w.Wp, w.W, sng, N, 1, 0, G2, N, w.wmax));
             if (!w.Bs.data)
-                JSTSP_TRY(hgemm_pack(ctx, w.Bs, ctx->arena, B, strideB, 1, G2, 0, G2, M, nB, (long long)G2 * M, w.Bc.bmax));
+                JSTSP_TRY(hgemm_pack(ctx, w.Bs, ctx->arena, B, strideB, 1, G2, 0, G2, M, nB, (long long)G2 * M, w.Bc.bmax, pack_gt));
             HGemmDesc hs{w.W, sng, N, w.wmax, w.Bs.data, strideB ? w.Bs.st : 0, w.Bs.bmax, strideB ? 1 : 0, w.Bs.KS,
                          w.Bs.JT, w.Xs, snm, N, N, M, G2, batch, fz ? EPI_UPDATE_C : EPI_NONE, w.prm, w.X, w.V2,
                          hmax ? w.nmax + 2 * (size_t)batch : nullptr, w.Wp.data, w.Wp.st, w.Wp.KS};
@@ -569,7 +596,7 @@
     }
 
     JSTSP_TRY(stage_out(ctx, reinterpret_cast<float2 *>(S_out), w.S, batch * g, memspace));
-    JSTSP_TRY(stage_out(ctx, reinterpret_cast<float2 *>(Y_out), w.Y, batch * nm, memspace));
+    if (!y_direct) JSTSP_TRY(stage_out(ctx, reinterpret_cast<float2 *>(Y_out), w.Y, batch * nm, memspace));
     if (want_ce && Imax > 0) JSTSP_TRY(stage_out(ctx, ce_out, w.ce, (size_t)batch * 3 * Imax, memspace));
     if (fusedp && overflowed) {
         std::vector<uint32_t> flags(batch);
diff --git a/jstsp19_amd/csrc/solver_common.h b/jstsp19_amd/csrc/solver_common.h
--- a/jstsp19_amd/csrc/solver_common.h
+++ b/jstsp19_amd/csrc/solver_common.h
@@ -151,7 +151,8 @@
 };
 bool fused_shape_ok(int N, int M, int G2, int parts);
 size_t fused_bytes(int M, int G2, int nB, int batch, int parts);
-int fused_probe_toeplitz(jstsp_ctx *ctx, Arena &ar, const float2 *B, long long sBt, int G2, int M, int nB, int *gt);
+int fused_probe_toeplitz(jstsp_ctx *ctx, Arena &ar, const float2 *B, long long sBt, int G2, int M, int nB, int *gt,
+                         uint32_t *bmax = nullptr, bool *bmax_valid = nullptr);
 int toeplitz_gram_assemble(jstsp_ctx *ctx, const float2 *B, long long sBt, int G2, int M, int gt, int nB, const float2 *G0,
                            const float2 *G0lo, float2 *G, float2 *Glo);
 int fused_alloc(Arena &ar, FusedWS &f, int M, int G2, int nB, int batch, int parts, int gt, int v2);
```
